# thu-pacman/chitu

Hardware: AMD Instinct MI355X
Metric: output tok/s (bs=16) DeepSeek-R1 FP8 TP=8; HBM GB/s vs peak (higher is better)
Workload: dtype fp8_e4m3 weights+activations (W8A8, fp32 accumulate), bf16 attention

## Files before the change

### chitu_amd/csrc/gate.hip

```cpp
#include "common.h"
#include "moe_align_device.h"

namespace chitu {

struct RouteAlign {
    int num_experts;
    int block_size;
    int32_t* sorted_ids;
    int64_t sorted_cap;
    int32_t* expert_ids;
    int64_t expert_cap;
    int32_t* num_post_pad;
    int32_t* cumsum;
    const int32_t* expert_map;
    unsigned int* ticket;
    int small;
};

__device__ __forceinline__ void route_align_tail(const RouteAlign& a, const int64_t* ids, int64_t numel, int* lds) {
    __shared__ int last_flag;
    asm volatile("s_waitcnt vmcnt(0)" ::: "memory");
    __syncthreads();
    if (gridDim.x == 1) {
        moe_align_workgroup<int64_t>(ids, numel, a.num_experts, a.block_size, a.sorted_ids, a.sorted_cap, a.expert_ids,
                                     a.expert_cap, a.num_post_pad, a.cumsum, 1, a.expert_map, lds, (int)blockDim.x);
        return;
    }
    if (threadIdx.x == 0) {
        __builtin_amdgcn_fence(__ATOMIC_RELEASE, "agent");
        asm volatile("s_waitcnt vmcnt(0)" ::: "memory");
        const unsigned int t = __hip_atomic_fetch_add(a.ticket, 1u, __ATOMIC_RELAXED, __HIP_MEMORY_SCOPE_AGENT);
        const int last = (t == gridDim.x - 1) ? 1 : 0;
        if (last) {
            __builtin_amdgcn_fence(__ATOMIC_ACQUIRE, "agent");
            __hip_atomic_store(a.ticket, 0u, __ATOMIC_RELAXED, __HIP_MEMORY_SCOPE_AGENT);
        }
        last_flag = last;
    }
    __syncthreads();
    if (!last_flag) return;
    moe_align_workgroup<int64_t>(ids, numel, a.num_experts, a.block_size, a.sorted_ids, a.sorted_cap, a.expert_ids,
                                 a.expert_cap, a.num_post_pad, a.cumsum, 1, a.expert_map, lds, (int)blockDim.x);
}

__device__ __forceinline__ float bf16r(float v) { return round_bf16(v); }

template <int SIGMOID>
__global__ __launch_bounds__(1024) void gate_route_kernel(
    const void* __restrict__ logits, int S, int M, int E, const bf16_t* __restrict__ bias, int n_groups,
    int topk_groups, int topk, float route_scale, bf16_t* __restrict__ out_w, int64_t* __restrict__ out_ids,
    int out_stride, int extra_id, float extra_w, int extra_n, int renorm, RouteAlign al) {
    extern __shared__ __attribute__((aligned(16))) float lds[];
    float* sc = lds;
    float* red = lds + E;
    float* gsc = lds + E + 32;
    float* wsel = lds + E + 32 + 64;
    const int t = blockIdx.x, e = threadIdx.x, lane = e & 63, wave = e >> 6;
    const int nw = blockDim.x >> 6;
    const bool act = e < E;

    float logit = -INFINITY;
    if (act) {
        if (S == 0) {
            logit = bf16_to_f32(((const bf16_t*)logits)[(int64_t)t * E + e]);
        } else {
            float a = 0.f;
            for (int s0 = 0; s0 < S; s0 += 8) {
                float v[8];
#pragma unroll
                for (int i = 0; i < 8; ++i)
                    v[i] = (s0 + i < S) ? ((const float*)logits)[((int64_t)(s0 + i) * M + t) * E + e] : 0.f;
#pragma unroll
                for (int i = 0; i < 8; ++i) a += v[i];
            }
            logit = bf16r(a);
        }
    }
    float orig;
    if (SIGMOID) {
        orig = act ? bf16r(1.0f / (1.0f + expf(-logit))) : 0.f;
    } else {
        float m = wave_reduce_max(logit);
        if (lane == 0) red[wave] = m;
        __syncthreads();
        m = red[0];
        for (int w = 1; w < nw; ++w) m = __builtin_fmaxf(m, red[w]);
        __syncthreads();
        const float ex = act ? expf(logit - m) : 0.f;
        float sum = wave_reduce_sum(ex);
        if (lane == 0) red[wave] = sum;
        __syncthreads();
        sum = 0.f;
        for (int w = 0; w < nw; ++w) sum += red[w];
        __syncthreads();
        orig = ex / sum;
    }
    float sel = orig;
    if (bias && act) sel = SIGMOID ? bf16r(orig + bf16_to_f32(bias[e])) : orig + bf16_to_f32(bias[e]);
    if (act) sc[e] = sel;
    __syncthreads();

    if (n_groups > 1) {
        const int gs = E / n_groups;
        if (gs == 32 || gs == 64) {
            const float v = act ? sel : -INFINITY;
            float m1 = v;
#pragma unroll
            for (int off = 1; off < 64; off <<= 1)
                if (off < gs) m1 = __builtin_fmaxf(m1, __shfl_xor(m1, off, 64));
            const unsigned long long gmask = gs == 64 ? ~0ull : (0xffffffffull << (lane & 32));
            const int n_max = __popcll(__ballot(v == m1) & gmask);
            float m2 = v < m1 ? v : -INFINITY;
#pragma unroll
            for (int off = 1; off < 64; off <<= 1)
                if (off < gs) m2 = __builtin_fmaxf(m2, __shfl_xor(m2, off, 64));
            if (n_max >= 2) m2 = m1;
            if (act && (e % gs) == 0) gsc[e / gs] = bias ? (SIGMOID ? bf16r(m1 + m2) : m1 + m2) : m1;
        } else if (e < n_groups) {
            float m1 = -INFINITY, m2 = -INFINITY;
            for (int i = 0; i < gs; ++i) {
                const float v = sc[e * gs + i];
                if (v > m1) { m2 = m1; m1 = v; }
                else if (v > m2) m2 = v;
            }
            gsc[e] = bias ? (SIGMOID ? bf16r(m1 + m2) : m1 + m2) : m1;
        }
        __syncthreads();
        if (act) {
            const int grp = e / gs;
            const float mine = gsc[grp];
            int rank = 0;
            for (int g2 = 0; g2 < n_groups; ++g2) {
                const float o = gsc[g2];
                rank += (o > mine) || (o == mine && g2 < grp);
            }
            if (rank >= topk_groups) sel = 0.f;
        }
        __syncthreads();
        if (act) sc[e] = sel;
        __syncthreads();
    }
    int rank = 0;
    if (act) {
        const int e4 = E & ~3;
#pragma unroll 16
        for (int i = 0; i < e4; i += 4) {
            const f32x4 o = *reinterpret_cast<const f32x4*>(&sc[i]);
            rank += (o[0] > sel) || (o[0] == sel && i < e);
            rank += (o[1] > sel) || (o[1] == sel && i + 1 < e);
            rank += (o[2] > sel) || (o[2] == sel && i + 2 < e);
            rank += (o[3] > sel) || (o[3] == sel && i + 3 < e);
        }
        for (int i = e4; i < E; ++i) {
            const float o = sc[i];
// ... 139 lines not shown
        if (lane < topk) {
            float sum = 0.f;
            for (int i = 0; i < topk; ++i) sum += wsel[i];
            float w = bf16r(wsel[lane] / bf16r(sum));
            w = bf16r(w * route_scale);
            out_w[(int64_t)t * out_stride + lane] = f32_to_bf16(w);
        }
        if (lane < extra_n && extra_id >= 0) {
            out_ids[(int64_t)t * out_stride + topk + lane] = extra_id + lane;
            out_w[(int64_t)t * out_stride + topk + lane] = f32_to_bf16(extra_w);
        }
    }
    if (al.num_experts > 0)
        route_align_tail(al, out_ids, (int64_t)M * out_stride, align_lds);
}

template <int GS>
__global__ __launch_bounds__(1024) void gate_route_align_wg_kernel(
    const void* __restrict__ logits, int S, int M, const bf16_t* __restrict__ bias, int n_groups, int topk_groups,
    int topk, float route_scale, bf16_t* __restrict__ out_w, int64_t* __restrict__ out_ids, int out_stride,
    int extra_id, float extra_w, int extra_n, RouteAlign al) {
    constexpr int E = 256;
    extern __shared__ __attribute__((aligned(16))) int dyn_lds[];
    const int nwaves = blockDim.x >> 6;
    float* orig_lds = reinterpret_cast<float*>(dyn_lds);
    int64_t* ids_lds = reinterpret_cast<int64_t*>(dyn_lds + nwaves * E);
    int* align_lds = dyn_lds + nwaves * E + 2 * ((M * out_stride + 1) & ~1);
    const int lane = threadIdx.x & 63, t = __builtin_amdgcn_readfirstlane(threadIdx.x >> 6);
    CHITU_PROBE_MARK(0);
    const bool small_sort = al.small != 0;
    if (small_sort) {
        moe_align_small_init(al.num_experts, (int64_t)M * out_stride, al.sorted_ids, al.sorted_cap, al.expert_ids, al.expert_cap,
                             align_lds, (int)threadIdx.x, (int)blockDim.x);
        __syncthreads();
    }
    if (t < M) {
        float lg[4];
        if (S == 0) {
            const i32x2 raw = *reinterpret_cast<const i32x2*>((const bf16_t*)logits + (int64_t)t * E + lane * 4);
            lg[0] = bf16_to_f32((bf16_t)((uint32_t)raw[0] & 0xffffu));
            lg[1] = bf16_to_f32((bf16_t)((uint32_t)raw[0] >> 16));
            lg[2] = bf16_to_f32((bf16_t)((uint32_t)raw[1] & 0xffffu));
            lg[3] = bf16_to_f32((bf16_t)((uint32_t)raw[1] >> 16));
        } else {
            f32x4 v[16];
#pragma unroll
            for (int i = 0; i < 16; ++i)
                v[i] = *reinterpret_cast<const f32x4*>((const float*)logits + ((int64_t)min(i, S - 1) * M + t) * E + lane * 4);
            f32x4 a = f32x4{0.f, 0.f, 0.f, 0.f};
#pragma unroll
            for (int i = 0; i < 16; ++i)
#pragma unroll
                for (int c = 0; c < 4; ++c) a[c] += i < S ? v[i][c] : 0.f;
#pragma unroll
            for (int c = 0; c < 4; ++c) lg[c] = bf16r(a[c]);
        }
        float bv[4] = {0.f, 0.f, 0.f, 0.f};
        if (bias) {
            const i32x2 raw = *reinterpret_cast<const i32x2*>(bias + lane * 4);
            bv[0] = bf16_to_f32((bf16_t)((uint32_t)raw[0] & 0xffffu));
            bv[1] = bf16_to_f32((bf16_t)((uint32_t)raw[0] >> 16));
            bv[2] = bf16_to_f32((bf16_t)((uint32_t)raw[1] & 0xffffu));
            bv[3] = bf16_to_f32((bf16_t)((uint32_t)raw[1] >> 16));
        }
        float orig[4], sel[4];
        uint32_t key[4];
        if (lg[0] == 12345.678f) CHITU_PROBE_MARK(9);
        CHITU_PROBE_MARK(1);
#pragma unroll
        for (int c = 0; c < 4; ++c) {
            orig[c] = bf16r(1.0f / (1.0f + expf(-lg[c])));
            sel[c] = bias ? bf16r(orig[c] + bv[c]) : orig[c];
            key[c] = score_key(sel[c], lane * 4 + c);
        }
        *reinterpret_cast<f32x4*>(&orig_lds[t * E + lane * 4]) = f32x4{orig[0], orig[1], orig[2], orig[3]};
        if (key[0] == 0xdeadbeefu) CHITU_PROBE_MARK(9);
        CHITU_PROBE_MARK(5);
        if (GS == 32) {
            const uint32_t k1 = group8_max_u32(max(max(key[0], key[1]), max(key[2], key[3])));
            uint32_t k2 = 0u;
#pragma unroll
            for (int c = 0; c < 4; ++c) k2 = max(k2, key[c] == k1 ? 0u : key[c]);
            k2 = group8_max_u32(k2);
            const float m1 = key_score(k1), m2 = key_score(k2);
            const float mine = bias ? bf16r(m1 + m2) : m1;
            const int grp = lane >> 3;
            int rank = 0;
#pragma unroll
            for (int g2 = 0; g2 < 8; ++g2) {
                const float o = __int_as_float(__builtin_amdgcn_readlane(__float_as_int(mine), g2 * 8));
                rank += (g2 < n_groups) && ((o > mine) || (o == mine && g2 < grp));
            }
            if (rank >= topk_groups) {
#pragma unroll
                for (int c = 0; c < 4; ++c) key[c] = score_key(0.f, lane * 4 + c);
            }
        }
        if (key[0] == 0xdeadbeefu) CHITU_PROBE_MARK(9);
        CHITU_PROBE_MARK(6);
        uint32_t mine_k = 0u;
        for (int r = 0; r < topk; ++r) {
            const uint32_t m = wave_max_u32_uniform(max(max(key[0], key[1]), max(key[2], key[3])));
            if (lane == r) mine_k = m;
#pragma unroll
            for (int c = 0; c < 4; ++c)
                if (key[c] == m) key[c] = 0u;
        }
        if (mine_k == 0xdeadbeefu) CHITU_PROBE_MARK(9);
        CHITU_PROBE_MARK(7);
        __builtin_amdgcn_fence(__ATOMIC_ACQ_REL, "wavefront");
        __builtin_amdgcn_wave_barrier();
        const int we = 0xffff - (int)(mine_k & 0xffffu);
        const float ws = lane < topk ? orig_lds[t * E + (we & (E - 1))] : 0.f;
        float sum = 0.f;
        if (topk <= 16) {
#pragma unroll
            for (int i = 0; i < 16; ++i)
                if (i < topk) sum += __int_as_float(__builtin_amdgcn_readlane(__float_as_int(ws), i));
        } else {
            for (int i = 0; i < topk; ++i) sum += __shfl(ws, i, 64);
        }
        if (lane < topk) {
            float w = bf16r(ws / bf16r(sum));
            w = bf16r(w * route_scale);
            out_w[(int64_t)t * out_stride + lane] = f32_to_bf16(w);
            out_ids[(int64_t)t * out_stride + lane] = we;
            ids_lds[t * out_stride + lane] = we;
            if (small_sort) moe_align_small_mark(align_lds, we, t);
        }
        if (lane < extra_n && extra_id >= 0) {
            out_ids[(int64_t)t * out_stride + topk + lane] = extra_id + lane;
            out_w[(int64_t)t * out_stride + topk + lane] = f32_to_bf16(extra_w);
            ids_lds[t * out_stride + topk + lane] = extra_id + lane;
            if (small_sort) moe_align_small_mark(align_lds, extra_id + lane, t);
        }
    }
    CHITU_PROBE_MARK(2);
    __syncthreads();
    CHITU_PROBE_MARK(3);
    const int sort_waves = min((int)(blockDim.x >> 6), max((al.num_experts + 63) >> 6, (M * out_stride + 63) >> 6));
    if (t >= sort_waves) return;
    if (small_sort) {
        moe_align_small_tail(ids_lds, M * out_stride, out_stride, al.num_experts, al.block_size, al.sorted_ids, al.sorted_cap,
                             al.expert_ids, al.expert_cap, al.num_post_pad, al.cumsum, al.expert_map, align_lds, sort_waves * 64);
        CHITU_PROBE_MARK(4);
        return;
    }
    moe_align_workgroup<int64_t>(ids_lds, (int64_t)M * out_stride, al.num_experts, al.block_size, al.sorted_ids,
                                 al.sorted_cap, al.expert_ids, al.expert_cap, al.num_post_pad, al.cumsum, 1,
                                 al.expert_map, align_lds, sort_waves * 64);
    CHITU_PROBE_MARK(4);
}

__device__ __forceinline__ uint32_t ordered_u32(float v) {
    const uint32_t b = __float_as_uint(v);
    return b ^ ((b & 0x80000000u) ? 0xffffffffu : 0x80000000u);
}

__global__ __launch_bounds__(1024) void gate_route_align_wg_softmax_kernel(
    const void* __restrict__ logits, int S, int M, int E, const bf16_t* __restrict__ bias, int topk, float route_scale,
    bf16_t* __restrict__ out_w, int64_t* __restrict__ out_ids, int out_stride, int extra_id, float extra_w, int extra_n,
    int renorm, RouteAlign al) {
    extern __shared__ __attribute__((aligned(16))) int dyn_lds[];
    int64_t* ids_lds = reinterpret_cast<int64_t*>(dyn_lds);
    int* align_lds = dyn_lds + 2 * ((M * out_stride + 1) & ~1);
    const int lane = threadIdx.x & 63, t = __builtin_amdgcn_readfirstlane(threadIdx.x >> 6);
    const bool small_sort = al.small != 0;
    if (small_sort) {
        moe_align_small_init(al.num_experts, (int64_t)M * out_stride, al.sorted_ids, al.sorted_cap, al.expert_ids, al.expert_cap,
                             align_lds, (int)threadIdx.x, (int)blockDim.x);
        __syncthreads();
    }
    if (t < M) {
        const bool act = lane < E;
        const int ec = act ? lane : E - 1;
        float logit;
        if (S == 0) {
            logit = bf16_to_f32(((const bf16_t*)logits)[(int64_t)t * E + ec]);
        } else {
            float v[16];
#pragma unroll
            for (int i = 0; i < 16; ++i) v[i] = ((const float*)logits)[((int64_t)min(i, S - 1) * M + t) * E + ec];
            float a = 0.f;
#pragma unroll
            for (int i = 0; i < 16; ++i) a += i < S ? v[i] : 0.f;
            logit = bf16r(a);
        }
        const float bv = bias ? bf16_to_f32(bias[ec]) : 0.f;
        if (!act) logit = -INFINITY;
        const float m = wave_reduce_max(logit);
        const float ex = act ? expf(logit - m) : 0.f;
        const float sum = wave_reduce_sum(ex);
        const float orig = ex / sum;
        const float sel = bias ? orig + bv : orig;
        uint32_t key = act ? ordered_u32(sel) : 0u;
        int my_e = 0;
        float my_w = 0.f;
        for (int r = 0; r < topk; ++r) {
            const uint32_t mk = wave_max_u32_uniform(key);
            const unsigned long long hit = __ballot(act && key == mk);
            const int win = __builtin_amdgcn_readfirstlane(__ffsll((long long)hit) - 1);
            const float w = __int_as_float(__builtin_amdgcn_readlane(__float_as_int(orig), win));
            if (lane == r) {
                my_e = win;
                my_w = w;
            }
            if (lane == win) key = 0u;
        }
        float w = my_w;
        if (renorm) {
            float s2 = 0.f;
#pragma unroll
            for (int i = 0; i < 16; ++i)
                if (i < topk) s2 += __int_as_float(__builtin_amdgcn_readlane(__float_as_int(my_w), i));
            w = w / s2;
        }
        w = w * route_scale;
        if (lane < topk) {
            out_w[(int64_t)t * out_stride + lane] = f32_to_bf16(w);
            out_ids[(int64_t)t * out_stride + lane] = my_e;
            ids_lds[t * out_stride + lane] = my_e;
            if (small_sort) moe_align_small_mark(align_lds, my_e, t);
        }
        if (lane < extra_n && extra_id >= 0) {
            out_ids[(int64_t)t * out_stride + topk + lane] = extra_id + lane;
            out_w[(int64_t)t * out_stride + topk + lane] = f32_to_bf16(extra_w);
            ids_lds[t * out_stride + topk + lane] = extra_id + lane;
            if (small_sort) moe_align_small_mark(align_lds, extra_id + lane, t);
        }
    }
    __syncthreads();
    const int sort_waves = min((int)(blockDim.x >> 6), max((al.num_experts + 63) >> 6, (M * out_stride + 63) >> 6));
    if (t >= sort_waves) return;
    if (small_sort) {
        moe_align_small_tail(ids_lds, M * out_stride, out_stride, al.num_experts, al.block_size, al.sorted_ids, al.sorted_cap,
                             al.expert_ids, al.expert_cap, al.num_post_pad, al.cumsum, al.expert_map, align_lds, sort_waves * 64);
        return;
    }
    moe_align_workgroup<int64_t>(ids_lds, (int64_t)M * out_stride, al.num_experts, al.block_size, al.sorted_ids,
                                 al.sorted_cap, al.expert_ids, al.expert_cap, al.num_post_pad, al.cumsum, 1,
                                 al.expert_map, align_lds, sort_waves * 64);
}

}

static int gate_route_launch(const void* logits, int32_t num_partials, int64_t tokens, int32_t num_experts,
                             const void* bias_bf16, int32_t n_groups, int32_t topk_groups, int32_t topk,
                             int32_t score_func, float route_scale, void* out_weights_bf16, int64_t* out_ids,
                             int32_t out_stride, int32_t extra_expert_id, float extra_weight,
                             int32_t extra_count, const chitu::RouteAlign& al, void* stream) {
    using namespace chitu;
    CHITU_REQUIRE(logits && out_weights_bf16 && out_ids && tokens >= 0);
    CHITU_REQUIRE(num_experts >= 1 && num_experts <= 1024 && topk >= 1 && topk <= num_experts && topk <= 64);
    CHITU_REQUIRE(n_groups >= 1 && n_groups <= 64 && num_experts % n_groups == 0);
    CHITU_REQUIRE(topk_groups >= 1 && topk_groups <= n_groups && num_partials >= 0);
    CHITU_REQUIRE(extra_count >= 0 && extra_count <= 32 && out_stride >= topk + (extra_expert_id >= 0 ? extra_count : 0));
    CHITU_REQUIRE(score_func >= 0 && score_func <= 2);
    if (tokens == 0) return CHITU_OK;
    const int threads = ((max(num_experts, al.num_experts) + 63) / 64) * 64;
    CHITU_REQUIRE(threads <= 1024);
    const size_t align_lds = al.num_experts > 0 ? sizeof(int) * moe_align_lds_ints(al.num_experts, threads) : 0;
    const size_t lds = max(sizeof(float) * (size_t)(num_experts + 32 + 64 + 64), align_lds);
    CHITU_REQUIRE(lds <= 60 * 1024);
    hipStream_t st = (hipStream_t)stream;
    const int gs = n_groups > 1 ? num_experts / n_groups : 0;
    const bool fast = score_func == 1 && (gs == 0 || gs == 32 || gs == 64) && num_partials <= 16 &&
                      (threads / 64) * topk <= 64 && ((threads / 64) * topk) % 4 == 0 && n_groups <= 32 &&
                      debug_option(kOptGateGeneric) <= 0;
    if (fast && al.num_experts > 0 && num_experts == 256 && (gs == 0 || gs == 32) && tokens <= 16 &&
        extra_count <= 32 && debug_option(kOptGateTicket) <= 0) {
        const int wg_threads = 64 * max((int)tokens, (max(num_experts, al.num_experts) + 63) / 64);
        const size_t ids_ints = 2 * (((size_t)tokens * out_stride + 1) & ~(size_t)1);
        const size_t wg_lds = sizeof(int) * ((size_t)(wg_threads / 64) * 256 + ids_ints +
                                             moe_align_lds_ints(al.num_experts, wg_threads));
        CHITU_REQUIRE(wg_threads <= 1024 && wg_lds <= 64 * 1024);
        RouteAlign alw = al;
        alw.small = (num_experts <= al.num_experts &&
                     (extra_expert_id < 0 || (extra_expert_id >= num_experts && extra_expert_id + extra_count <= al.num_experts)) &&
                     debug_option(kOptGateSmallSort) != 0) ? 1 : 0;
#define LAUNCHW(GSV)                                                                                          \
    hipLaunchKernelGGL(gate_route_align_wg_kernel<GSV>, dim3(1), dim3(wg_threads), wg_lds, st, logits,         \
                       (int)num_partials, (int)tokens, (const bf16_t*)bias_bf16, (int)n_groups, (int)topk_groups, \
                       (int)topk, route_scale, (bf16_t*)out_weights_bf16, out_ids, (int)out_stride,           \
                       (int)extra_expert_id, extra_weight, (int)extra_count, alw)
        if (gs == 32) LAUNCHW(32);
        else LAUNCHW(0);
#undef LAUNCHW
        CHITU_RETURN_LAUNCH_STATUS();
    }
    if (!fast && al.num_experts > 0 && num_experts <= 64 && (score_func == 0 || score_func == 2) && n_groups <= 1 &&
        tokens <= 16 && num_partials <= 16 && topk <= 16 && extra_count <= 32 && debug_option(kOptGateTicket) <= 0 &&
        debug_option(kOptGateGeneric) <= 0) {
        const int wg_threads = 64 * max((int)tokens, (max(num_experts, al.num_experts) + 63) / 64);
        const size_t ids_ints = 2 * (((size_t)tokens * out_stride + 1) & ~(size_t)1);
        const size_t wg_lds = sizeof(int) * (ids_ints + moe_align_lds_ints(al.num_experts, wg_threads));
        CHITU_REQUIRE(wg_threads <= 1024 && wg_lds <= 64 * 1024);
        RouteAlign alw = al;
        alw.small = (num_experts <= al.num_experts &&
                     (extra_expert_id < 0 || (extra_expert_id >= num_experts && extra_expert_id + extra_count <= al.num_experts)) &&
                     debug_option(kOptGateSmallSort) != 0) ? 1 : 0;
        hipLaunchKernelGGL(gate_route_align_wg_softmax_kernel, dim3(1), dim3(wg_threads), wg_lds, st, logits, (int)num_partials,
                           (int)tokens, (int)num_experts, (const bf16_t*)bias_bf16, (int)topk, route_scale,
                           (bf16_t*)out_weights_bf16, out_ids, (int)out_stride, (int)extra_expert_id, extra_weight,
                           (int)extra_count, score_func == 2 ? 1 : 0, alw);
        CHITU_RETURN_LAUNCH_STATUS();
    }
    if (fast) {
#define LAUNCHF(GSV)                                                                                         \
    hipLaunchKernelGGL(gate_route_fast_kernel<GSV>, dim3((unsigned)tokens), dim3(threads), align_lds, st, logits, \
                       (int)num_partials, (int)tokens, (int)num_experts, (const bf16_t*)bias_bf16, (int)n_groups, \
                       (int)topk_groups, (int)topk, route_scale, (bf16_t*)out_weights_bf16, out_ids,         \
                       (int)out_stride, (int)extra_expert_id, extra_weight, (int)extra_count, al)
        if (gs == 32) LAUNCHF(32);
        else if (gs == 64) LAUNCHF(64);
        else LAUNCHF(0);
#undef LAUNCHF
        CHITU_RETURN_LAUNCH_STATUS();
    }
    if (lds > 48 * 1024) {
        (void)hipFuncSetAttribute((const void*)gate_route_kernel<1>, hipFuncAttributeMaxDynamicSharedMemorySize, (int)lds);
        (void)hipFuncSetAttribute((const void*)gate_route_kernel<0>, hipFuncAttributeMaxDynamicSharedMemorySize, (int)lds);
    }
    if (score_func == 1)
        hipLaunchKernelGGL(gate_route_kernel<1>, dim3((unsigned)tokens), dim3(threads), lds, st, logits,
                           (int)num_partials, (int)tokens, (int)num_experts, (const bf16_t*)bias_bf16,
                           (int)n_groups, (int)topk_groups, (int)topk, route_scale, (bf16_t*)out_weights_bf16,
                           out_ids, (int)out_stride, (int)extra_expert_id, extra_weight, (int)extra_count, 0, al);
    else
        hipLaunchKernelGGL(gate_route_kernel<0>, dim3((unsigned)tokens), dim3(threads), lds, st, logits,
                           (int)num_partials, (int)tokens, (int)num_experts, (const bf16_t*)bias_bf16,
                           (int)n_groups, (int)topk_groups, (int)topk, route_scale, (bf16_t*)out_weights_bf16,
                           out_ids, (int)out_stride, (int)extra_expert_id, extra_weight, (int)extra_count,
                           score_func == 2 ? 1 : 0, al);
    CHITU_RETURN_LAUNCH_STATUS();
}

extern "C" int chitu_hip_gate_route(const void* logits, int32_t num_partials, int64_t tokens,
                                    int32_t num_experts, const void* bias_bf16, int32_t n_groups,
                                    int32_t topk_groups, int32_t topk, int32_t score_func,
                                    float route_scale, void* out_weights_bf16, int64_t* out_ids,
                                    int32_t out_stride, int32_t extra_expert_id, float extra_weight,
                                    int32_t extra_count, void* stream) {
    chitu::RouteAlign none{};
    return gate_route_launch(logits, num_partials, tokens, num_experts, bias_bf16, n_groups, topk_groups, topk,
                             score_func, route_scale, out_weights_bf16, out_ids, out_stride, extra_expert_id,
                             extra_weight, extra_count, none, stream);
}

extern "C" int chitu_hip_gate_route_align(const void* logits, int32_t num_partials, int64_t tokens,
                                          int32_t num_experts, const void* bias_bf16, int32_t n_groups,
                                          int32_t topk_groups, int32_t topk, int32_t score_func,
                                          float route_scale, void* out_weights_bf16, int64_t* out_ids,
                                          int32_t out_stride, int32_t extra_expert_id, float extra_weight,
                                          int32_t extra_count, int32_t align_num_experts, int32_t align_block_size,
                                          int32_t* sorted_token_ids, int64_t sorted_cap, int32_t* expert_ids,
                                          int64_t expert_ids_cap, int32_t* num_tokens_post_pad, int32_t* cumsum,
                                          const int32_t* expert_map, uint32_t* ticket, void* stream) {
    CHITU_REQUIRE(sorted_token_ids && expert_ids && num_tokens_post_pad && cumsum && ticket);
    CHITU_REQUIRE(align_num_experts >= 1 && align_num_experts <= 1024 && align_block_size >= 1);
    CHITU_REQUIRE(sorted_cap >= 0 && expert_ids_cap >= 0 && tokens * (int64_t)out_stride < (1ll << 31));
    CHITU_REQUIRE(out_stride == topk + (extra_expert_id >= 0 ? extra_count : 0));
    chitu::RouteAlign al{align_num_experts, align_block_size, sorted_token_ids, sorted_cap, expert_ids, expert_ids_cap,
                         num_tokens_post_pad, cumsum, expert_map, ticket, 0};
    return gate_route_launch(logits, num_partials, tokens, num_experts, bias_bf16, n_groups, topk_groups, topk,
                             score_func, route_scale, out_weights_bf16, out_ids, out_stride, extra_expert_id,
                             extra_weight, extra_count, al, stream);
}

CHITU_PROBE_READER(gate)
```

### chitu_amd/csrc/moe.hip

```cpp
#include "common.h"
#include "gemm_common.h"
#ifndef CHITU_MOE_PROBE_MASK
#define CHITU_MOE_PROBE_MASK 0
#endif

namespace chitu {

struct MoeStage {
    W8Frag w;
    i32x4 x[2];
    float xs, ws;
};


template <int WK, int NW, int D>
__global__ __launch_bounds__(64 * WK * NW) void moe_gemm1_kernel(
    const fp8_t* __restrict__ Xq, const float* __restrict__ Xs, const fp8_t* __restrict__ W,
    const float* __restrict__ Ws, const int32_t* __restrict__ sorted_ids,
    const int32_t* __restrict__ expert_ids, const int32_t* __restrict__ num_post_pad,
    bf16_t* __restrict__ out, int numel, int topk, int N, int K) {
    static_assert(WK == 1 || NW == 1, "either split K or tile N inside a workgroup");
    __shared__ float red[WK > 1 ? WK * 256 : 1];
    const int mb = blockIdx.y;
    if (mb * 16 >= *num_post_pad) return;
    const int lane = threadIdx.x & 63, wave = __builtin_amdgcn_readfirstlane(threadIdx.x >> 6);
    const int j = lane & 15, g = lane >> 4;
    const int n0 = (NW > 1 ? blockIdx.x * NW + wave : blockIdx.x) * 16;
    if (NW > 1 && n0 >= N) return;
    const int KB = K >> 7;
    const int slot = sorted_ids[mb * 16 + j];
    const bool valid = slot < numel;
    const int e = expert_ids[mb];
    f32x4 acc = f32x4{0.f, 0.f, 0.f, 0.f};
    if (e >= 0) {
        const int kw = NW > 1 ? 0 : wave;
        const int kb0 = KB * kw / WK, kb1 = KB * (kw + 1) / WK;
        const int slot0 = __builtin_amdgcn_readfirstlane(slot);
        const int token = (valid ? slot : min(slot0, numel - 1)) / topk;
        const fp8_t* xp = Xq + (size_t)token * K + g * 16;
        const float* xsp = Xs + (size_t)token * KB;
        const fp8_t *wp0, *wp1;
        w8_lane_ptrs(W + (size_t)e * N * K, n0, N, K, j, g, wp0, wp1);
        const float* wsp = Ws + ((size_t)e * ((N + 127) >> 7) + (n0 >> 7)) * KB;
        auto load = [&](MoeStage& st, int kb) {
            const int off = kb << 7;
            st.w.w[0] = __builtin_nontemporal_load(reinterpret_cast<const i32x4*>(wp0 + off));
            st.w.w[1] = __builtin_nontemporal_load(reinterpret_cast<const i32x4*>(wp1 + off));
            st.x[0] = *reinterpret_cast<const i32x4*>(xp + off);
            st.x[1] = *reinterpret_cast<const i32x4*>(xp + off + 64);
            st.xs = xsp[kb];
            st.ws = wsp[kb];
        };
        auto compute = [&](const MoeStage& st) {
            const f32x4 blk = w8a8_block_dot(st.w, st.x[0], st.x[1]);
#pragma unroll
            for (int r = 0; r < 4; ++r) acc[r] += (blk[r] * st.xs) * st.ws;
        };
        MoeStage ring[D];
#pragma unroll
        for (int d = 0; d < D; ++d)
            if (kb0 + d < kb1) load(ring[d], kb0 + d);
        for (int kb = kb0; kb < kb1; kb += D) {
#pragma unroll
            for (int d = 0; d < D; ++d) {
                if (kb + d < kb1) {
                    compute(ring[d]);
                    if (kb + d + D < kb1) load(ring[d], kb + d + D);
                }
            }
        }
    }
    if (WK > 1) {
        *reinterpret_cast<f32x4*>(&red[(wave * 64 + lane) * 4]) = acc;
        __syncthreads();
        if (wave != 0) return;
        acc = f32x4{0.f, 0.f, 0.f, 0.f};
#pragma unroll
        for (int w = 0; w < WK; ++w) {
            const f32x4 v = *reinterpret_cast<const f32x4*>(&red[(w * 64 + lane) * 4]);
#pragma unroll
            for (int r = 0; r < 4; ++r) acc[r] += v[r];
        }
    }
    if (!valid) return;
    moe_store_tile(out + (size_t)slot * N, n0, g, N, acc, 1.0f);
}

struct MoeStage2 {
    W8Frag wg, wu;
    i32x4 x[2];
    float xs, wsg, wsu;
};

template <int WK, int D, bool Q = false>
__global__ __launch_bounds__(Q ? 512 : 64 * WK) void moe_gemm1_silu_kernel(
    const fp8_t* __restrict__ Xq, const float* __restrict__ Xs, const fp8_t* __restrict__ W,
    const float* __restrict__ Ws, const int32_t* __restrict__ sorted_ids,
    const int32_t* __restrict__ expert_ids, const int32_t* __restrict__ num_post_pad,
    bf16_t* __restrict__ out, int numel, int topk, int I, int K, fp8_t* __restrict__ hq = nullptr,
    float* __restrict__ hs = nullptr, float eps = 0.f) {
    static_assert(!Q || WK == 1, "the quantising epilogue owns whole K");
    __shared__ float red[WK > 1 ? WK * 512 : 1];
    __shared__ float qmax[Q ? 8 * 16 : 1];
    const int mb = blockIdx.y;
    if (mb * 16 >= *num_post_pad) return;
    const int lane = threadIdx.x & 63;
    const int wave_id = __builtin_amdgcn_readfirstlane(threadIdx.x >> 6);
    const int wave = Q ? 0 : wave_id;
    const int j = lane & 15, g = lane >> 4;
    const int n0 = (Q ? blockIdx.x * 8 + wave_id : blockIdx.x) * 16;
    const int N = 2 * I;
    const int KB = K >> 7;
    const int slot = sorted_ids[mb * 16 + j];
    const bool valid = slot < numel;
    const int e = expert_ids[mb];
    f32x4 ag = f32x4{0.f, 0.f, 0.f, 0.f}, au = f32x4{0.f, 0.f, 0.f, 0.f};
    if (e >= 0) {
        const int kb0 = KB * wave / WK, kb1 = KB * (wave + 1) / WK;
        const int slot0 = __builtin_amdgcn_readfirstlane(slot);
        const int token = (valid ? slot : min(slot0, numel - 1)) / topk;
        const fp8_t* xp = Xq + (size_t)token * K + g * 16;
        const float* xsp = Xs + (size_t)token * KB;
        if (CHITU_MOE_PROBE_MASK & 1) {
            xp = Xq + (size_t)(g * 16 + (token & 15)) * 16;
            xsp = Xs + (token & 15);
        }
        const fp8_t* Wb = W + (size_t)e * N * K;
        const fp8_t *gp0, *gp1, *up0, *up1;
        w8_lane_ptrs(Wb, n0, N, K, j, g, gp0, gp1);
        w8_lane_ptrs(Wb, I + n0, N, K, j, g, up0, up1);
        const float* wsb = Ws + (size_t)e * ((N + 127) >> 7) * KB;
        const float* wsgp = wsb + (size_t)(n0 >> 7) * KB;
        const float* wsup = wsb + (size_t)((I + n0) >> 7) * KB;
        auto load = [&](MoeStage2& st, int kb) {
            const int off = kb << 7;
            st.wg.w[0] = __builtin_nontemporal_load(reinterpret_cast<const i32x4*>(gp0 + off));
            st.wg.w[1] = __builtin_nontemporal_load(reinterpret_cast<const i32x4*>(gp1 + off));
            st.wu.w[0] = __builtin_nontemporal_load(reinterpret_cast<const i32x4*>(up0 + off));
            st.wu.w[1] = __builtin_nontemporal_load(reinterpret_cast<const i32x4*>(up1 + off));
            if (CHITU_MOE_PROBE_MASK & 1) {
                st.x[0] = *reinterpret_cast<const i32x4*>(xp + (size_t)kb * 2048);
                st.x[1] = *reinterpret_cast<const i32x4*>(xp + (size_t)kb * 2048 + 1024);
                st.xs = xsp[kb * 16];
            } else {
                st.x[0] = *reinterpret_cast<const i32x4*>(xp + off);
                st.x[1] = *reinterpret_cast<const i32x4*>(xp + off + 64);
                st.xs = xsp[kb];
            }
            st.wsg = wsgp[kb];
            st.wsu = wsup[kb];
        };
        auto compute = [&](const MoeStage2& st) {
            const f32x4 bg = w8a8_block_dot(st.wg, st.x[0], st.x[1]);
            const f32x4 bu = w8a8_block_dot(st.wu, st.x[0], st.x[1]);
#pragma unroll
            for (int r = 0; r < 4; ++r) {
                ag[r] += (bg[r] * st.xs) * st.wsg;
                au[r] += (bu[r] * st.xs) * st.wsu;
            }
        };
        MoeStage2 ring[D];
#pragma unroll
        for (int d = 0; d < D; ++d)
            if (kb0 + d < kb1) load(ring[d], kb0 + d);
        for (int kb = kb0; kb < kb1; kb += D) {
#pragma unroll
            for (int d = 0; d < D; ++d) {
                if (kb + d < kb1) {
                    compute(ring[d]);
                    if (kb + d + D < kb1) load(ring[d], kb + d + D);
                }
            }
        }
    }
    if (WK > 1) {
        *reinterpret_cast<f32x4*>(&red[(wave * 128 + lane) * 4]) = ag;
        *reinterpret_cast<f32x4*>(&red[(wave * 128 + 64 + lane) * 4]) = au;
        __syncthreads();
        if (wave != 0) return;
        ag = f32x4{0.f, 0.f, 0.f, 0.f};
        au = f32x4{0.f, 0.f, 0.f, 0.f};
#pragma unroll
        for (int w = 0; w < WK; ++w) {
            const f32x4 vg = *reinterpret_cast<const f32x4*>(&red[(w * 128 + lane) * 4]);
            const f32x4 vu = *reinterpret_cast<const f32x4*>(&red[(w * 128 + 64 + lane) * 4]);
#pragma unroll
            for (int r = 0; r < 4; ++r) {
                ag[r] += vg[r];
                au[r] += vu[r];
            }
        }
    }
    if (!Q && !valid) return;
    f32x4 h;
#pragma unroll
    for (int r = 0; r < 4; ++r) {
        const float gv = round_bf16(ag[r]), uv = round_bf16(au[r]);
        const float sl = round_bf16(gv / (1.0f + expf(-gv)));
        h[r] = round_bf16(sl * uv);
    }
    if (!Q) {
        moe_store_tile(out + (size_t)slot * I, n0, g, I, h, 1.0f);
        return;
    }
    float amax = __builtin_fmaxf(__builtin_fmaxf(__builtin_fabsf(h[0]), __builtin_fabsf(h[1])),
                                 __builtin_fmaxf(__builtin_fabsf(h[2]), __builtin_fabsf(h[3])));
    amax = __builtin_fmaxf(amax, __shfl_xor(amax, 16, 64));
    amax = __builtin_fmaxf(amax, __shfl_xor(amax, 32, 64));
    if (g == 0) qmax[wave_id * 16 + j] = amax;
    __syncthreads();
    amax = qmax[j];
#pragma unroll
    for (int w = 1; w < 8; ++w) amax = __builtin_fmaxf(amax, qmax[w * 16 + j]);
    const float sc = __builtin_fmaxf(amax, eps) / 448.0f;
    const float v[8] = {h[0], h[1], h[2], h[3], 0.f, 0.f, 0.f, 0.f};
    const uint32_t codes = (uint32_t)quant8_fp8<true>(v, sc)[0];
    if (!valid) return;
    fp8_t* qrow = hq + (size_t)slot * I + n0 + 2 * g;
    *reinterpret_cast<uint16_t*>(qrow) = (uint16_t)(codes & 0xffffu);
    *reinterpret_cast<uint16_t*>(qrow + 8) = (uint16_t)(codes >> 16);
    if (wave_id == 0 && g == 0) hs[(size_t)slot * (I >> 7) + blockIdx.x] = sc;
}

__global__ __launch_bounds__(256) void moe_silu_quant_kernel(const bf16_t* __restrict__ c1,
                                                             fp8_t* __restrict__ q,
                                                             float* __restrict__ s, int64_t rows,
                                                             int I, float eps, int act_rule) {
    const int lane16 = threadIdx.x & 15;
    const int gpr = I >> 7;
    const int64_t n_groups = rows * gpr;
    int64_t group = ((int64_t)blockIdx.x * blockDim.x + threadIdx.x) >> 4;
    const int64_t stride = ((int64_t)gridDim.x * blockDim.x) >> 4;
    for (; group < n_groups; group += stride) {
        const int64_t row = group / gpr;
        const int col = (int)(group % gpr) * 128 + lane16 * 8;
        const i32x4 graw = *reinterpret_cast<const i32x4*>(c1 + row * 2 * I + col);
        const i32x4 uraw = *reinterpret_cast<const i32x4*>(c1 + row * 2 * I + I + col);
        float h[8];
        float amax = 0.f;
#pragma unroll
        for (int i = 0; i < 8; ++i) {
            const uint32_t gu = (uint32_t)graw[i >> 1], uu = (uint32_t)uraw[i >> 1];
            const float gv = (i & 1) ? __uint_as_float(gu & 0xffff0000u) : __uint_as_float(gu << 16);
            const float uv = (i & 1) ? __uint_as_float(uu & 0xffff0000u) : __uint_as_float(uu << 16);
            const float sl = round_bf16(gv / (1.0f + expf(-gv)));
            h[i] = round_bf16(sl * uv);
            amax = __builtin_fmaxf(amax, __builtin_fabsf(h[i]));
        }
        amax = row16_reduce_max(amax);
        if (!act_rule) amax = __builtin_fmaxf(amax, eps);
        const float sc = amax / 448.0f;
        const i32x2 o = act_rule ? quant8_fp8<false>(h, sc) : quant8_fp8<true>(h, sc);
        *reinterpret_cast<i32x2*>(q + row * I + col) = o;
        if (lane16 == 0) s[group] = sc;
    }
}

template <int KBMAX, int NT>
__global__ __launch_bounds__(256) void moe_gemm2_kernel(
    const fp8_t* __restrict__ Hq, const float* __restrict__ Hs, const fp8_t* __restrict__ W,
    const float* __restrict__ Ws, const int32_t* __restrict__ sorted_ids,
    const int32_t* __restrict__ expert_ids, const int32_t* __restrict__ num_post_pad,
    const void* __restrict__ topk_w, int w_dt, bf16_t* __restrict__ out, int numel, int N, int I,
    int mul_weight) {
    const int mb = blockIdx.y;
    if (mb * 16 >= *num_post_pad) return;
    const int lane = threadIdx.x & 63, wave = __builtin_amdgcn_readfirstlane(threadIdx.x >> 6);
    const int j = lane & 15, g = lane >> 4;
    const int KB = I >> 7;
    const int slot = sorted_ids[mb * 16 + j];
    const bool valid = slot < numel;
    const int e = expert_ids[mb];
    const int row = valid ? slot : 0;
    const float rw = (mul_weight && valid) ? moe_routed_weight(topk_w, w_dt, slot) : 1.0f;
    i32x4 x[KBMAX][2];
    float xs[KBMAX];
    if (e >= 0) {
        const fp8_t* xp = Hq + (size_t)row * I + g * 16;
#pragma unroll
        for (int kb = 0; kb < KBMAX; ++kb) {
            if (kb < KB) {
                x[kb][0] = *reinterpret_cast<const i32x4*>(xp + (kb << 7));
                x[kb][1] = *reinterpret_cast<const i32x4*>(xp + (kb << 7) + 64);
                xs[kb] = Hs[(size_t)row * KB + kb];
            }
        }
    }
    const int tile0 = (blockIdx.x * 4 + wave) * NT;
    W8Frag wf[NT][KBMAX];
    if (e >= 0) {
#pragma unroll
        for (int t = 0; t < NT; ++t) {
            const int n0 = (tile0 + t) * 16;
            if (n0 < N) {
                const fp8_t *wp0, *wp1;
                w8_lane_ptrs(W + (size_t)e * N * I, n0, N, I, j, g, wp0, wp1);
#pragma unroll
                for (int kb = 0; kb < KBMAX; ++kb) {
                    if (kb < KB) {
                        wf[t][kb].w[0] = __builtin_nontemporal_load(reinterpret_cast<const i32x4*>(wp0 + (kb << 7)));
                        wf[t][kb].w[1] = __builtin_nontemporal_load(reinterpret_cast<const i32x4*>(wp1 + (kb << 7)));
                    }
                }
            }
        }
    }
#pragma unroll
    for (int t = 0; t < NT; ++t) {
        const int n0 = (tile0 + t) * 16;
        if (n0 >= N) break;
        f32x4 acc = f32x4{0.f, 0.f, 0.f, 0.f};
        if (e >= 0) {
            const float* wsp = Ws + ((size_t)e * ((N + 127) >> 7) + (n0 >> 7)) * KB;
#pragma unroll
            for (int kb = 0; kb < KBMAX; ++kb) {
                if (kb < KB) {
                    const f32x4 blk = w8a8_block_dot(wf[t][kb], x[kb][0], x[kb][1]);
                    const float ws = wsp[kb];
#pragma unroll
                    for (int r = 0; r < 4; ++r) acc[r] += (blk[r] * xs[kb]) * ws;
                }
            }
        }
        if (valid) moe_store_tile(out + (size_t)slot * N, n0, g, N, acc, rw);
    }
}

template <int KB, int NT, int ROUNDS>
__global__ __launch_bounds__(256) void moe_gemm2_q_kernel(
    const bf16_t* __restrict__ Hb, const fp8_t* __restrict__ W, const float* __restrict__ Ws,
    const int32_t* __restrict__ sorted_ids, const int32_t* __restrict__ expert_ids,
    const int32_t* __restrict__ num_post_pad, const void* __restrict__ topk_w, int w_dt,
    bf16_t* __restrict__ out, int numel, int N, int mul_weight, float eps) {
    constexpr int I = KB * 128;
    constexpr int HPW = (2 * KB + 3) / 4;
    __shared__ float amax_lds[2 * KB][16];
    __shared__ i32x4 xq_lds[2 * KB][64];
    const int mb = blockIdx.y;
    if (mb * 16 >= *num_post_pad) return;
    const int lane = threadIdx.x & 63, wave = __builtin_amdgcn_readfirstlane(threadIdx.x >> 6);
    const int j = lane & 15, g = lane >> 4;
    const int slot = sorted_ids[mb * 16 + j];
    const bool valid = slot < numel;
    const int e = expert_ids[mb];
    auto tile_of = [&](int r) { return ((blockIdx.x * ROUNDS + r) * 4 + wave) * NT; };
    if (e < 0) {
#pragma unroll
        for (int r = 0; r < ROUNDS; ++r)
#pragma unroll
            for (int t = 0; t < NT; ++t) {
                const int n0 = (tile_of(r) + t) * 16;
                if (n0 < N && valid) moe_store_tile(out + (size_t)slot * N, n0, g, N, f32x4{0.f, 0.f, 0.f, 0.f}, 1.0f);
            }
        return;
    }
    const int row = valid ? slot : 0;
    const bf16_t* hrow = Hb + (size_t)row * I;
    i32x4 hraw[HPW][2];
#pragma unroll
    for (int q = 0; q < HPW; ++q) {
        const int hb = min(wave + 4 * q, 2 * KB - 1);
        hraw[q][0] = *reinterpret_cast<const i32x4*>(hrow + hb * 64 + g * 16);
        hraw[q][1] = *reinterpret_cast<const i32x4*>(hrow + hb * 64 + g * 16 + 8);
    }
    const int last_tile = (N - 1) >> 4;
    const fp8_t* We = W + (size_t)e * N * I;
    W8Frag wf[ROUNDS > 1 ? 2 : 1][NT][KB];
    auto load_round = [&](W8Frag (&dst)[NT][KB], int r) {
#pragma unroll
        for (int t = 0; t < NT; ++t) {
            const int n0 = min(tile_of(r) + t, last_tile) * 16;
            const fp8_t *wp0, *wp1;
            w8_lane_ptrs(We, n0, N, I, j, g, wp0, wp1);
#pragma unroll
            for (int kb = 0; kb < KB; ++kb) {
                dst[t][kb].w[0] = __builtin_nontemporal_load(reinterpret_cast<const i32x4*>(wp0 + (kb << 7)));
                dst[t][kb].w[1] = __builtin_nontemporal_load(reinterpret_cast<const i32x4*>(wp1 + (kb << 7)));
            }
        }
    };
    load_round(wf[0], 0);
    const float rw = (mul_weight && valid) ? moe_routed_weight(topk_w, w_dt, slot) : 1.0f;
    float h[HPW][16];
#pragma unroll
    for (int q = 0; q < HPW; ++q) {
        const int hb = wave + 4 * q;
        float amax = 0.f;
#pragma unroll
        for (int i = 0; i < 16; ++i) {
            const uint32_t u = (uint32_t)hraw[q][i >> 3][(i >> 1) & 3];
            h[q][i] = (i & 1) ? __uint_as_float(u & 0xffff0000u) : __uint_as_float(u << 16);
            amax = __builtin_fmaxf(amax, __builtin_fabsf(h[q][i]));
        }
        amax = __builtin_fmaxf(amax, __shfl_xor(amax, 16, 64));
        amax = __builtin_fmaxf(amax, __shfl_xor(amax, 32, 64));
        if (g == 0 && hb < 2 * KB) amax_lds[hb][j] = amax;
    }
    __syncthreads();
#pragma unroll
    for (int q = 0; q < HPW; ++q) {
        const int hb = wave + 4 * q;
        if (hb < 2 * KB) {
            const float sc = __builtin_fmaxf(__builtin_fmaxf(amax_lds[hb & ~1][j], amax_lds[hb | 1][j]), eps) / 448.0f;
            float lo[8], hi[8];
#pragma unroll
            for (int i = 0; i < 8; ++i) {
                lo[i] = h[q][i];
                hi[i] = h[q][8 + i];
            }
            const i32x2 a = quant8_fp8<true>(lo, sc), b = quant8_fp8<true>(hi, sc);
            xq_lds[hb][lane] = i32x4{a[0], a[1], b[0], b[1]};
        }
    }
    __syncthreads();
    i32x4 x[KB][2];
    float xs[KB];
#pragma unroll
    for (int kb = 0; kb < KB; ++kb) {
        x[kb][0] = xq_lds[2 * kb][lane];
        x[kb][1] = xq_lds[2 * kb + 1][lane];
        xs[kb] = __builtin_fmaxf(__builtin_fmaxf(amax_lds[2 * kb][j], amax_lds[2 * kb + 1][j]), eps) / 448.0f;
    }
    const float* wse = Ws + (size_t)e * ((N + 127) >> 7) * KB;
#pragma unroll
    for (int r = 0; r < ROUNDS; ++r) {
        if (r + 1 < ROUNDS) load_round(wf[(r + 1) & 1], r + 1);
#pragma unroll
        for (int t = 0; t < NT; ++t) {
            const int n0 = (tile_of(r) + t) * 16;
            f32x4 acc = f32x4{0.f, 0.f, 0.f, 0.f};
            const float* wsp = wse + (size_t)(min(n0, N - 1) >> 7) * KB;
#pragma unroll
            for (int kb = 0; kb < KB; ++kb) {
                const f32x4 blk = w8a8_block_dot(wf[r & 1][t][kb], x[kb][0], x[kb][1]);
                const float ws = wsp[kb];
#pragma unroll
                for (int rr = 0; rr < 4; ++rr) acc[rr] += (blk[rr] * xs[kb]) * ws;
            }
            if (valid && n0 < N) moe_store_tile(out + (size_t)slot * N, n0, g, N, acc, rw);
        }
    }
}

template <int WK>
__global__ __launch_bounds__(64 * WK) void moe_gemm2_generic_kernel(
    const fp8_t* __restrict__ Hq, const float* __restrict__ Hs, const fp8_t* __restrict__ W,
    const float* __restrict__ Ws, const int32_t* __restrict__ sorted_ids,
    const int32_t* __restrict__ expert_ids, const int32_t* __restrict__ num_post_pad,
    const void* __restrict__ topk_w, int w_dt, bf16_t* __restrict__ out, int numel, int N, int I,
    int mul_weight) {
    __shared__ float red[WK > 1 ? WK * 256 : 1];
    const int mb = blockIdx.y;
    if (mb * 16 >= *num_post_pad) return;
    const int lane = threadIdx.x & 63, wave = __builtin_amdgcn_readfirstlane(threadIdx.x >> 6);
    const int j = lane & 15, g = lane >> 4;
    const int n0 = blockIdx.x * 16;
    const int KB = I >> 7;
    const int slot = sorted_ids[mb * 16 + j];
    const bool valid = slot < numel;
    const int e = expert_ids[mb];
    const int row = valid ? slot : 0;
    f32x4 acc = f32x4{0.f, 0.f, 0.f, 0.f};
    if (e >= 0) {
        const int kb0 = KB * wave / WK, kb1 = KB * (wave + 1) / WK;
        const fp8_t* xp = Hq + (size_t)row * I + g * 16;
        const float* xsp = Hs + (size_t)row * KB;
        const fp8_t *wp0, *wp1;
        w8_lane_ptrs(W + (size_t)e * N * I, n0, N, I, j, g, wp0, wp1);
        const float* wsp = Ws + ((size_t)e * ((N + 127) >> 7) + (n0 >> 7)) * KB;
        for (int kb = kb0; kb < kb1; ++kb) {
            const int off = kb << 7;
            W8Frag f;
            f.w[0] = __builtin_nontemporal_load(reinterpret_cast<const i32x4*>(wp0 + off));
            f.w[1] = __builtin_nontemporal_load(reinterpret_cast<const i32x4*>(wp1 + off));
            const i32x4 x0 = *reinterpret_cast<const i32x4*>(xp + off);
            const i32x4 x1 = *reinterpret_cast<const i32x4*>(xp + off + 64);
            const f32x4 blk = w8a8_block_dot(f, x0, x1);
            const float xs = xsp[kb], ws = wsp[kb];
#pragma unroll
            for (int r = 0; r < 4; ++r) acc[r] += (blk[r] * xs) * ws;
        }
    }
    if (WK > 1) {
        *reinterpret_cast<f32x4*>(&red[(wave * 64 + lane) * 4]) = acc;
        __syncthreads();
        if (wave != 0) return;
        acc = f32x4{0.f, 0.f, 0.f, 0.f};
#pragma unroll
        for (int w = 0; w < WK; ++w) {
            const f32x4 v = *reinterpret_cast<const f32x4*>(&red[(w * 64 + lane) * 4]);
#pragma unroll
            for (int r = 0; r < 4; ++r) acc[r] += v[r];
        }
    }
    if (!valid) return;
    const float rw = mul_weight ? moe_routed_weight(topk_w, w_dt, slot) : 1.0f;
    moe_store_tile(out + (size_t)slot * N, n0, g, N, acc, rw);
}

__global__ __launch_bounds__(256) void moe_sum_kernel(const bf16_t* __restrict__ c3,
                                                      bf16_t* __restrict__ out, int64_t M, int topk,
                                                      int64_t N) {
    const int64_t n8 = N >> 3;
    for (int64_t idx = (int64_t)blockIdx.x * blockDim.x + threadIdx.x; idx < M * n8;
         idx += (int64_t)gridDim.x * blockDim.x) {
        const int64_t t = idx / n8, c = (idx % n8) * 8;
        float acc[8] = {0.f, 0.f, 0.f, 0.f, 0.f, 0.f, 0.f, 0.f};
        for (int k = 0; k < topk; ++k) {
// ... 57 lines not shown
#undef LAUNCH
    CHITU_RETURN_LAUNCH_STATUS();
}

extern "C" int chitu_hip_moe_silu_mul_quant_fp8(const void* c1_bf16, int64_t rows,
                                                int64_t inter_size, int32_t quant_mode, float eps,
                                                void* q_fp8, float* scales, void* stream) {
    using namespace chitu;
    CHITU_REQUIRE(c1_bf16 && q_fp8 && scales && rows >= 0 && inter_size >= 128);
    CHITU_REQUIRE(quant_mode == 0 || quant_mode == 1);
    if (inter_size % 128 != 0) return CHITU_ERR_UNSUPPORTED;
    if (rows == 0) return CHITU_OK;
    const int64_t lanes = rows * (inter_size / 128) * 16;
    int64_t blocks = (lanes + 255) / 256;
    if (blocks > 2048) blocks = 2048;
    hipLaunchKernelGGL(moe_silu_quant_kernel, dim3((unsigned)blocks), dim3(256), 0,
                       (hipStream_t)stream, (const bf16_t*)c1_bf16, (fp8_t*)q_fp8, scales, rows,
                       (int)inter_size, eps, quant_mode == 0 ? 1 : 0);
    CHITU_RETURN_LAUNCH_STATUS();
}

extern "C" int chitu_hip_moe_gemm2_fp8(const void* h_fp8, const float* h_scale, const void* w2_fp8,
                                       const float* w2_scale, const int32_t* sorted_token_ids,
                                       const int32_t* expert_ids,
                                       const int32_t* num_tokens_post_pad, const void* topk_weights,
                                       int weights_dtype, int32_t mul_routed_weight,
                                       void* out_bf16, int64_t numel, int64_t N, int64_t inter_size,
                                       int64_t max_mblocks, void* stream) {
    using namespace chitu;
    CHITU_REQUIRE(h_fp8 && h_scale && w2_fp8 && w2_scale && sorted_token_ids && expert_ids);
    CHITU_REQUIRE(num_tokens_post_pad && out_bf16 && (topk_weights || !mul_routed_weight));
    CHITU_REQUIRE(numel >= 0 && N >= 1 && inter_size >= 128 && max_mblocks >= 0);
    CHITU_REQUIRE(weights_dtype >= 0 && weights_dtype <= 2);
    if (inter_size % 128 != 0) return CHITU_ERR_UNSUPPORTED;
    if (numel == 0 || max_mblocks == 0) return CHITU_OK;
    hipStream_t st = (hipStream_t)stream;
    const int n_tiles = (int)((N + 15) / 16);
    const int KB = (int)(inter_size / 128);
    if (KB <= 4) {
        const int64_t mbs = numel < max_mblocks ? numel : max_mblocks;
#define LAUNCH2(KBM, NTV)                                                                        \
    hipLaunchKernelGGL((moe_gemm2_kernel<KBM, NTV>),                                             \
                       dim3((unsigned)((n_tiles + 4 * NTV - 1) / (4 * NTV)), (unsigned)max_mblocks), \
                       dim3(256), 0, st, (const fp8_t*)h_fp8, h_scale, (const fp8_t*)w2_fp8,     \
                       w2_scale, sorted_token_ids, expert_ids, num_tokens_post_pad, topk_weights, \
                       weights_dtype, (bf16_t*)out_bf16, (int)numel, (int)N, (int)inter_size,    \
                       (int)mul_routed_weight)
        const bool many = (int64_t)n_tiles * mbs > 8192;
        if (KB <= 2) {
            if (many) LAUNCH2(2, 4); else LAUNCH2(2, 2);
        } else {
            if (many) LAUNCH2(4, 4); else LAUNCH2(4, 2);
        }
#undef LAUNCH2
    } else {
        const dim3 grid((unsigned)n_tiles, (unsigned)max_mblocks);
        const int64_t wgs = (int64_t)n_tiles * (numel < max_mblocks ? numel : max_mblocks);
        int WK = wgs <= 512 ? 8 : wgs <= 1024 ? 4 : wgs <= 4096 ? 2 : 1;
        while (WK > 1 && WK > KB) WK >>= 1;
#define LAUNCHG(WKV)                                                                              \
    hipLaunchKernelGGL(moe_gemm2_generic_kernel<WKV>, grid, dim3(64 * WKV), 0, st,                \
                       (const fp8_t*)h_fp8, h_scale, (const fp8_t*)w2_fp8, w2_scale,              \
                       sorted_token_ids, expert_ids, num_tokens_post_pad, topk_weights,           \
                       weights_dtype, (bf16_t*)out_bf16, (int)numel, (int)N, (int)inter_size,     \
                       (int)mul_routed_weight)
        switch (WK) {
            case 8: LAUNCHG(8); break;
            case 4: LAUNCHG(4); break;
            case 2: LAUNCHG(2); break;
            default: LAUNCHG(1); break;
        }
#undef LAUNCHG
    }
    CHITU_RETURN_LAUNCH_STATUS();
}

extern "C" int chitu_hip_moe_gemm1_silu_fp8(const void* a_fp8, const float* a_scale, const void* w1_fp8,
                                            const float* w1_scale, const int32_t* sorted_token_ids,
                                            const int32_t* expert_ids, const int32_t* num_tokens_post_pad,
                                            void* h_bf16, int64_t numel, int32_t topk, int64_t inter_size,
                                            int64_t K, int64_t max_mblocks, void* stream) {
    using namespace chitu;
    CHITU_REQUIRE(a_fp8 && a_scale && w1_fp8 && w1_scale && sorted_token_ids && expert_ids);
    CHITU_REQUIRE(num_tokens_post_pad && h_bf16);
    CHITU_REQUIRE(numel >= 0 && topk >= 1 && inter_size >= 16 && K >= 128 && max_mblocks >= 0);
    if (K % 128 != 0 || inter_size % 16 != 0) return CHITU_ERR_UNSUPPORTED;
    if (numel == 0 || max_mblocks == 0) return CHITU_OK;
    const int n_tiles = (int)(inter_size / 16);
    const int64_t wgs = 2 * (int64_t)n_tiles * (numel < max_mblocks ? numel : max_mblocks);
    const int KB = (int)(K / 128);
    int WK = wgs <= 640 ? 8 : wgs <= 1536 ? 4 : wgs <= 3200 ? 2 : 1;
    debug_override(kOptMoeGemm1WK, WK);
    while (WK > 1 && WK > KB) WK >>= 1;
    int D = WK >= 4 ? 2 : 3;
    debug_override(kOptMoeGemm1D, D);
    hipStream_t st = (hipStream_t)stream;
    const dim3 grid((unsigned)n_tiles, (unsigned)max_mblocks);
#define LAUNCH1S(WKV, DV)                                                                                     \
    hipLaunchKernelGGL((moe_gemm1_silu_kernel<WKV, DV>), grid, dim3(64 * WKV), 0, st, (const fp8_t*)a_fp8, a_scale, \
                       (const fp8_t*)w1_fp8, w1_scale, sorted_token_ids, expert_ids, num_tokens_post_pad,      \
                       (bf16_t*)h_bf16, (int)numel, (int)topk, (int)inter_size, (int)K)
    if (WK == 8) { if (D == 2) LAUNCH1S(8, 2); else if (D == 3) LAUNCH1S(8, 3); else LAUNCH1S(8, 4); }
    else if (WK == 4) { if (D == 2) LAUNCH1S(4, 2); else if (D == 3) LAUNCH1S(4, 3); else LAUNCH1S(4, 4); }
    else if (WK == 2) { if (D == 4) LAUNCH1S(2, 4); else LAUNCH1S(2, 3); }
    else { if (D == 4) LAUNCH1S(1, 4); else LAUNCH1S(1, 3); }
#undef LAUNCH1S
    CHITU_RETURN_LAUNCH_STATUS();
}

extern "C" int chitu_hip_moe_gemm2_quant_fp8(const void* h_bf16, const void* w2_fp8, const float* w2_scale,
                                             const int32_t* sorted_token_ids, const int32_t* expert_ids,
                                             const int32_t* num_tokens_post_pad, const void* topk_weights,
                                             int weights_dtype, int32_t mul_routed_weight, void* out_bf16,
                                             int64_t numel, int64_t N, int64_t inter_size, int64_t max_mblocks,
                                             float eps, void* stream) {
    using namespace chitu;
    CHITU_REQUIRE(h_bf16 && w2_fp8 && w2_scale && sorted_token_ids && expert_ids);
    CHITU_REQUIRE(num_tokens_post_pad && out_bf16 && (topk_weights || !mul_routed_weight));
    CHITU_REQUIRE(numel >= 0 && N >= 1 && inter_size >= 128 && max_mblocks >= 0);
    CHITU_REQUIRE(weights_dtype >= 0 && weights_dtype <= 2);
    if (inter_size % 128 != 0 || inter_size > 512) return CHITU_ERR_UNSUPPORTED;
    if (numel == 0 || max_mblocks == 0) return CHITU_OK;
    hipStream_t st = (hipStream_t)stream;
    const int n_tiles = (int)((N + 15) / 16);
    const int KB = (int)(inter_size / 128);
    const int64_t mbs = numel < max_mblocks ? numel : max_mblocks;
#define LAUNCH2Q(KBV, NTV, RV)                                                                       \
    hipLaunchKernelGGL((moe_gemm2_q_kernel<KBV, NTV, RV>),                                           \
                       dim3((unsigned)((n_tiles + 4 * NTV * RV - 1) / (4 * NTV * RV)), (unsigned)max_mblocks), \
                       dim3(256), 0, st, (const bf16_t*)h_bf16, (const fp8_t*)w2_fp8, w2_scale,      \
                       sorted_token_ids, expert_ids, num_tokens_post_pad, topk_weights, weights_dtype, \
                       (bf16_t*)out_bf16, (int)numel, (int)N, (int)mul_routed_weight, eps)
    const bool many = (int64_t)n_tiles * mbs > 50000;
    int cfg = many ? 24 : 21;
    debug_override(kOptMoeGemm2Cfg, cfg);
    switch (KB) {
        case 1: LAUNCH2Q(1, 2, 1); break;
        case 2:
            if (cfg == 42) LAUNCH2Q(2, 4, 2);
            else if (cfg == 44) LAUNCH2Q(2, 4, 4);
            else if (cfg == 22) LAUNCH2Q(2, 2, 2);
            else if (cfg == 24) LAUNCH2Q(2, 2, 4);
            else if (cfg == 28) LAUNCH2Q(2, 2, 8);
            else if (cfg == 21) LAUNCH2Q(2, 2, 1);
            else LAUNCH2Q(2, 4, 1);
            break;
        case 3: LAUNCH2Q(3, 2, 1); break;
        default: LAUNCH2Q(4, 2, 1); break;
    }
#undef LAUNCH2Q
    CHITU_RETURN_LAUNCH_STATUS();
}

extern "C" int chitu_hip_moe_sum(const void* c3_bf16, void* out_bf16, int64_t tokens, int32_t topk,
                                 int64_t N, void* stream) {
    using namespace chitu;
    CHITU_REQUIRE(c3_bf16 && out_bf16 && tokens >= 0 && topk >= 1 && N >= 8);
    if (N % 8 != 0) return CHITU_ERR_UNSUPPORTED;
    if (tokens == 0) return CHITU_OK;
    int64_t blocks = (tokens * (N / 8) + 255) / 256;
    if (blocks > 2048) blocks = 2048;
    hipLaunchKernelGGL(moe_sum_kernel, dim3((unsigned)blocks), dim3(256), 0, (hipStream_t)stream,
                       (const bf16_t*)c3_bf16, (bf16_t*)out_bf16, tokens, (int)topk, N);
    CHITU_RETURN_LAUNCH_STATUS();
}
```

### chitu_amd/csrc/moe_align_device.h

```cpp
#pragma once
#include "common.h"

namespace chitu {

__host__ __device__ inline size_t moe_align_lds_ints(int E, int nthreads) {
    const int W = nthreads / 64;
    return (size_t)2 * E + W + (size_t)W * E;
}

template <typename id_t>
__device__ __forceinline__ void moe_align_workgroup(
    const id_t* __restrict__ ids, int64_t numel, int E, int block_size,
    int32_t* __restrict__ sorted_ids, int64_t sorted_cap, int32_t* __restrict__ expert_ids,
    int64_t expert_cap, int32_t* __restrict__ num_post_pad, int32_t* __restrict__ cumsum,
    int fill, const int32_t* __restrict__ expert_map, int* lds, const int nthreads) {
    const int nwaves = nthreads >> 6;
    int* counts = lds;
    int* cursor = lds + E;
    int* wave_tot = lds + 2 * E;
    int* wave_hist = lds + 2 * E + nwaves;

    const int tid = threadIdx.x;
    const int lane = tid & 63;
    const int wave = __builtin_amdgcn_readfirstlane(tid >> 6);
// ... 17 lines not shown
#pragma unroll
        for (int u = 0; u < 4; ++u)
            if (e4[u] >= 0 && e4[u] < E) atomicAdd(&my_hist[(int)e4[u]], 1);
    }
    __syncthreads();
    CHITU_PROBE_MARK(21);

    int padded = 0;
    if (tid < E) {
        int total = 0;
        for (int w = 0; w < nwaves; ++w) total += wave_hist[w * E + tid];
        counts[tid] = total;
        padded = ((total + block_size - 1) / block_size) * block_size;
    }
    int incl = padded;
#pragma unroll
    for (int off = 1; off < 64; off <<= 1) {
        const int up = __shfl_up(incl, off, 64);
        if (lane >= off) incl += up;
    }
    if (lane == 63) wave_tot[wave] = incl;
    __syncthreads();
    int wave_base = 0;
    for (int w = 0; w < wave; ++w) wave_base += wave_tot[w];
    incl += wave_base;
    const int start = incl - padded;
    if (tid < E) {
        const int32_t own_id = expert_map ? expert_map[tid] : (int32_t)tid;
        int run = start;
        for (int w = 0; w < nwaves; ++w) {
            const int c = wave_hist[w * E + tid];
            wave_hist[w * E + tid] = run;
            run += c;
        }
        cursor[tid] = run;
        cumsum[tid + 1] = incl;
        for (int i = start; i < incl; i += block_size) {
            const int b = i / block_size;
            if (b < expert_cap) expert_ids[b] = own_id;
        }
        if (tid == E - 1) *num_post_pad = incl;
    }
    if (tid == 0) cumsum[0] = 0;
    if (expert_map) {
        int total = 0;
        for (int w = 0; w < nwaves; ++w) total += wave_tot[w];
        const int32_t tail_id = expert_map[0];
        for (int64_t b = total / block_size + tid; b < expert_cap; b += nthreads) expert_ids[b] = tail_id;
    }
    __syncthreads();
    CHITU_PROBE_MARK(22);

    int nbits = 0;
    while ((1 << nbits) < E) ++nbits;
    for (int64_t base4 = w0; base4 < w1; base4 += 256) {
        int64_t e4[4];
#pragma unroll
        for (int u = 0; u < 4; ++u) e4[u] = base4 + 64 * u + lane < w1 ? (int64_t)ids[base4 + 64 * u + lane] : -1;
#pragma unroll
        for (int u = 0; u < 4; ++u) {
            const int64_t base = base4 + 64 * u;
            if (base >= w1) break;
            const int64_t i = base + lane;
            const int64_t e64 = e4[u];
            const bool valid = (e64 >= 0 && e64 < E);
            const int e = valid ? (int)e64 : 0;

            unsigned long long same = __ballot(valid);
            for (int b = 0; b < nbits; ++b) {
                const bool bit = (e >> b) & 1;
                const unsigned long long bal = __ballot(valid && bit);
                same &= bit ? bal : ~bal;
            }
            const unsigned long long lt = (lane == 0) ? 0ull : (~0ull >> (64 - lane));
            const int rank = __popcll(same & lt);
            int pos = 0;
            if (valid) pos = my_hist[e] + rank;
            __builtin_amdgcn_wave_barrier();
            if (valid) {
                if (rank == 0) my_hist[e] = pos + __popcll(same);
                if (pos < sorted_cap) sorted_ids[pos] = (int32_t)i;
            }
            __builtin_amdgcn_wave_barrier();
        }
    }
}

__host__ __device__ inline size_t moe_align_small_lds_ints(int E, int nthreads) { return (size_t)2 * E + nthreads / 64; }

__device__ __forceinline__ void moe_align_small_init(int E, int64_t numel, int32_t* __restrict__ sorted_ids, int64_t sorted_cap,
                                                     int32_t* __restrict__ expert_ids, int64_t expert_cap, int* lds,
                                                     int tid, int nthreads) {
    for (int i = tid; i < E; i += nthreads) lds[i] = 0;
    for (int64_t i = tid; i < sorted_cap; i += nthreads) sorted_ids[i] = (int32_t)numel;
    for (int64_t i = tid; i < expert_cap; i += nthreads) expert_ids[i] = 0;
}

__device__ __forceinline__ void moe_align_small_mark(int* lds, int e, int token) { atomicOr(&lds[e], 1 << token); }

__device__ __forceinline__ void moe_align_small_tail(
    const int64_t* __restrict__ ids_lds, int numel, int stride, int E, int block_size, int32_t* __restrict__ sorted_ids,
    int64_t sorted_cap, int32_t* __restrict__ expert_ids, int64_t expert_cap, int32_t* __restrict__ num_post_pad,
    int32_t* __restrict__ cumsum, const int32_t* __restrict__ expert_map, int* lds, const int nthreads) {
    const int nwaves = nthreads >> 6;
    int* tmask = lds;
    int* start_l = lds + E;
    int* wave_tot = lds + 2 * E;
    const int tid = threadIdx.x, lane = tid & 63;
    const int wave = __builtin_amdgcn_readfirstlane(tid >> 6);
    int padded = 0;
    if (tid < E) padded = ((__popc((unsigned)tmask[tid]) + block_size - 1) / block_size) * block_size;
    int incl = padded;
#pragma unroll
    for (int off = 1; off < 64; off <<= 1) {
        const int up = __shfl_up(incl, off, 64);
        if (lane >= off) incl += up;
    }
    if (lane == 63) wave_tot[wave] = incl;
    __syncthreads();
    int wave_base = 0, total = 0;
    for (int w = 0; w < nwaves; ++w) {
        const int t = wave_tot[w];
        if (w < wave) wave_base += t;
        total += t;
    }
    incl += wave_base;
    const int start = incl - padded;
    if (tid < E) {
        const int32_t own_id = expert_map ? expert_map[tid] : (int32_t)tid;
        start_l[tid] = start;
        cumsum[tid + 1] = incl;
        for (int i = start; i < incl; i += block_size) {
            const int b = i / block_size;
            if (b < expert_cap) expert_ids[b] = own_id;
        }
        if (tid == E - 1) *num_post_pad = incl;
    }
    if (tid == 0) cumsum[0] = 0;
    if (expert_map) {
        const int32_t tail_id = expert_map[0];
        for (int64_t b = total / block_size + tid; b < expert_cap; b += nthreads) expert_ids[b] = tail_id;
    }
    __syncthreads();
    if (tid < numel) {
        const int e = (int)ids_lds[tid];
        const int t = tid / stride;
        if (e >= 0 && e < E) {
            const int pos = start_l[e] + __popc((unsigned)tmask[e] & ((1u << t) - 1u));
            if (pos >= 0 && pos < sorted_cap) sorted_ids[pos] = (int32_t)tid;
        }
    }
}

}
```

### chitu_amd/deepseek_v3.py

```python

import math
from dataclasses import dataclass
from typing import List, Optional

import os

import torch
import torch.nn.functional as F

from . import fused_moe, graphs, ops
from . import tensor_parallel as tp
from .attn_backend import MLA_MULTI_MAX_Q, HipAttnBackend
from .cache_manager import MAX_DECODE_Q, PagedKVCacheManager, mla_kv_layout

FP8 = torch.float8_e4m3fn
BLOCK = 128


@dataclass
class DeepSeekV3Args:

    vocab_size: int = 129280
    dim: int = 7168
    inter_dim: int = 18432
# ... 187 lines not shown
        return self._w_uk_t

    def first_projection(self):
        return self.wqkv_a if self.q_lora_rank > 0 else self.wq_kv_a

    def decode_forward_paged(self, x_quant, cos, sin, first=None, q_len=1):
        H, C, R = self.n_local_heads, self.kv_lora_rank, self.qk_rope_head_dim
        if first is not None:
            bs = first.shape[0]
        else:
            bs = x_quant[0].rows if isinstance(x_quant[0], ops.TiledQuant) else x_quant[0].shape[0]
        cache = self.cache
        kv_cache = cache.get_paged_kv_cache(self.layer_id)
        if q_len > 1:
            assert bs % q_len == 0
            kv_table, kv_lens = cache.get_gpu_multi_block_table(), cache.get_gpu_multi_row_lens()
        else:
            kv_table, kv_lens = cache.get_gpu_block_table(), cache.get_gpu_seq_lens_excl_this_decode()
        paged = None
        if self.kv_fp8:
            paged = (kv_cache, kv_table, kv_lens)
            kv_cache, kv_table, kv_lens = self.kv_stage.rows, self.kv_stage.table[:bs], self.kv_stage.lens[:bs]
        nblk = C // BLOCK
        if self.q_lora_rank > 0:
            splits = _wqkv_a_splits(bs, self.wqkv_a.out_features, self.wqkv_a.in_features)
            if first is not None or isinstance(x_quant[0], ops.TiledQuant):
                splits = 1
            if first is not None:
                q_a_kv = first
            elif splits > 1:
                q_a_kv = ops.fp8_gemm_partials_deepseek_v3(x_quant[0], x_quant[1], self.wqkv_a.weight, self.wqkv_a.scale, splits)
            else:
                q_a_kv = self.wqkv_a(None, x_quant=x_quant)
            if FUSE_Q_PROJ and splits == 1 and bs <= _Q_PROJ_MAX_BS and ops.mla_q_proj_fits(bs, self.q_lora_rank):
                q = ops.mla_q_proj(q_a_kv, self.q_lora_rank, self.q_norm.weight, self.q_norm.eps, self.wq_b.weight,
                                   self.wq_b.scale, self.kv_norm.weight, self.kv_norm.eps, cos, sin, kv_cache,
                                   kv_table, kv_lens, out_dtype=torch.bfloat16)
            else:
                qq, qs = ops.mla_qkv_post(q_a_kv, self.q_lora_rank, self.q_norm.weight, self.q_norm.eps, self.kv_norm.weight,
                                          self.kv_norm.eps, cos, sin, kv_cache, kv_table, kv_lens)
                q = self.wq_b(None, x_quant=(qq, qs))
            q = q.view(bs, H, self.qk_head_dim)
            q_nope, q_pe = q[..., : self.qk_nope_head_dim], q[..., self.qk_nope_head_dim :]
            q_abs = ops.absorb_bmm_rope_fp8(q_nope, self.w_uk_transposed(), self.wkv_b.scale, 0, 2 * nblk, 1, 0, q_pe, cos, sin)
        else:
            q_kv = first if first is not None else self.wq_kv_a(None, x_quant=x_quant)
            nq = H * self.qk_head_dim
            q = q_kv[:, :nq].view(bs, H, self.qk_head_dim)
            q_nope, q_pe = q[..., : self.qk_nope_head_dim], q[..., self.qk_nope_head_dim :]
            q_abs = ops.absorb_bmm_rope_kv_fp8(q_nope, self.w_uk_transposed(), self.wkv_b.scale, 0, 2 * nblk, 1, 0, q_pe, cos, sin,
                                               q_kv[:, nq:], self.kv_norm.weight, self.kv_norm.eps, kv_cache,
                                               kv_table, kv_lens)
        if paged is not None:
            kv_cache = paged[0]
            ops.append_mla_kv_fp8(kv_cache, paged[1], self.kv_stage.rows[:bs], paged[2])
        fuse_merge = bs <= 32 and C == 512
        w_uv = self.wkv_b.weight.view(H, self.qk_nope_head_dim + self.v_head_dim, C)[:, self.qk_nope_head_dim :]
        if q_len == 1 and fuse_merge and _MLA_FUSED_TAIL and self.v_head_dim == 128:
            fused = self.attn_backend.mla_decode_merge_uv_quant(
                q_abs, q_pe, kv_cache, cache.get_gpu_seq_lens_incl_this_decode(), cache.get_gpu_block_table(), self.softmax_scale,
                w_uv, self.wkv_b.scale, nblk, 2 * nblk, 1, tile_major=ops.tile_major_ok(bs))
            if fused is not None:
                return self.wo(None, x_quant=fused)
        if q_len > 1:
            o = self.attn_backend.mla_decode_multi(q_abs.view(bs // q_len, q_len, H, C), q_pe.unflatten(0, (bs // q_len, q_len)), kv_cache,
                                                   cache.get_gpu_multi_seq_lens_incl(), cache.get_gpu_multi_block_table()[::q_len],
                                                   self.softmax_scale, return_partials=fuse_merge,
                                                   expanded=(cache.get_gpu_multi_block_table(), cache.get_gpu_multi_row_lens_incl()))
            if not isinstance(o, tuple):
                o = o.view(bs, H, C)
        else:
            o = self.attn_backend.mla_decode(q_abs, q_pe, kv_cache, cache.get_gpu_seq_lens_incl_this_decode(),
                                             cache.get_gpu_block_table(), self.softmax_scale, return_partials=fuse_merge)
        if isinstance(o, tuple):
            oq, os_ = ops.mla_merge_absorb_uv_quant_fp8(o[0], o[1], bs, w_uv, self.wkv_b.scale, nblk, 2 * nblk, 1,
                                                        tile_major=ops.tile_major_ok(bs))
        else:
            oq, os_ = ops.absorb_uv_quant_fp8(o, w_uv, self.wkv_b.scale, nblk, 2 * nblk, 1)
        return self.wo(None, x_quant=(oq, os_))


    def prefill_forward(self, x_quant, cos, sin, varlens):
        if getattr(varlens, "continued", False):
            return self.prefill_forward_paged(x_quant, cos, sin, varlens)
        H, C, R = self.n_local_heads, self.kv_lora_rank, self.qk_rope_head_dim
        T = x_quant[0].shape[0]
        q_abs, q_pe, kv_c, kv_pe = self._prefill_projections(x_quant, cos, sin)
        self.cache.finalize_cache_bylayer_prefill(ops.mla_kv_quant_fp8(kv_pe) if self.kv_fp8 else kv_pe, None,
                                                  self.cache.curr_req_ids, self.cache.curr_varlens, self.layer_id)
        o = self.attn_backend.attn_varlen_func(
            torch.cat([q_abs, q_pe], dim=-1), kv_pe.view(T, 1, C + R), kv_c.view(T, 1, C), varlens.prefix_lens,
            varlens.prefix_lens, varlens.max_len, varlens.max_len, causal=True, softmax_scale=self.softmax_scale)
        return self._prefill_output(o)

    def _prefill_projections(self, x_quant, cos, sin):
        H, C = self.n_local_heads, self.kv_lora_rank
        T = x_quant[0].shape[0]
        if self.q_lora_rank > 0:
            q_a_kv = self.wqkv_a(None, x_quant=x_quant)
            ql = self.q_lora_rank
            _, qq, qs = ops.rms_norm(q_a_kv[:, :ql], self.q_norm.weight, self.q_norm.eps, out_bf16=False, quant="act")
            q = self.wq_b(None, x_quant=(qq, qs)).view(T, H, self.qk_head_dim)
        else:
            q_a_kv = self.wq_kv_a(None, x_quant=x_quant)
            ql = H * self.qk_head_dim
            q = q_a_kv[:, :ql].view(T, H, self.qk_head_dim)
        q_nope, q_pe = q[..., : self.qk_nope_head_dim], q[..., self.qk_nope_head_dim :]
        kv_c = ops.rms_norm(q_a_kv[:, ql : ql + C], self.kv_norm.weight, self.kv_norm.eps)
        q_pe, k_pe = ops.apply_rotary_pos_emb(q_pe, q_a_kv[:, ql + C :], cos, sin, rotary_type="llama")
        kv_pe = torch.cat([kv_c, k_pe], dim=-1)
        nblk = C // BLOCK
        q_abs = ops.absorb_bmm_fp8(q_nope, self.w_uk_transposed(), self.wkv_b.scale, 0, 2 * nblk, 1, 0)
        return q_abs, q_pe, kv_c, kv_pe

    def _prefill_output(self, o):
        H, C = self.n_local_heads, self.kv_lora_rank
        nblk = C // BLOCK
        w_uv = self.wkv_b.weight.view(H, self.qk_nope_head_dim + self.v_head_dim, C)[:, self.qk_nope_head_dim :]
        oq, os_ = ops.absorb_uv_quant_fp8(o, w_uv, self.wkv_b.scale, nblk, 2 * nblk, 1)
        return self.wo(None, x_quant=(oq, os_))

    def prefill_forward_paged(self, x_quant, cos, sin, varlens):
        q_abs, q_pe, _, kv_pe = self._prefill_projections(x_quant, cos, sin)
        self.cache.finalize_cache_bylayer_prefill_continue(ops.mla_kv_quant_fp8(kv_pe) if self.kv_fp8 else kv_pe, None, self.layer_id)
        o = self.attn_backend.mla_attn_varlen_with_kvcache(
            torch.cat([q_abs, q_pe], dim=-1), self.cache.get_paged_kv_cache(self.layer_id), varlens.prefix_lens,
            self.cache.get_gpu_continue_seq_lens_incl(), self.cache.get_gpu_continue_block_table(), varlens.max_len,
            varlens.total_keys, self.softmax_scale, gathered=varlens.gathered)
        return self._prefill_output(o)


class MLPDeepSeekV3(torch.nn.Module):

    def __init__(self, args, device=None, inter: Optional[int] = None):
        super().__init__()
        tp_size = args.tp_degree()
        self.inter = args.inter_dim // tp_size if inter is None else inter
        self.w1w3 = Fp8Linear(args.dim, 2 * self.inter, device)
        self.w2 = Fp8Linear(self.inter, args.dim, device)

    def forward(self, x_quant):
        h = self.w1w3(None, x_quant=x_quant)
        hq, hs = fused_moe.silu_and_mul_quant(h, mode="act")
        return self.w2(None, x_quant=(hq, hs))


_ROUTE_ALIGN_MAX_TOKENS = 64


def _route_align_enabled(tokens: int) -> bool:
    return tokens <= _ROUTE_ALIGN_MAX_TOKENS and os.environ.get("CHITU_ROUTE_ALIGN", "1") != "0"


class GateDeepSeekV3(torch.nn.Module):

    def __init__(self, args, device=None):
        super().__init__()
        self.topk, self.n_groups, self.topk_groups = args.n_activated_experts, args.n_expert_groups, args.n_limited_groups
        self.score_func, self.route_scale = args.score_func, args.route_scale
        self.weight = torch.nn.Parameter(torch.empty(args.n_routed_experts, args.dim, dtype=torch.bfloat16, device=device), requires_grad=False)
        self.bias = (torch.nn.Parameter(torch.empty(args.n_routed_experts, dtype=torch.bfloat16, device=device), requires_grad=False)
                     if args.has_gate_bias() else None)

    def forward(self, x, extra_expert_id: int = -1, extra_count: int = 1, align=None, logits_partials=None):
        return ops.gate_deepseek_v3(x, self.weight, self.bias, self.n_groups, self.topk_groups, self.topk,
                                    self.score_func, self.route_scale, extra_expert_id=extra_expert_id,
                                    extra_count=extra_count, align=align, logits_partials=logits_partials)


class MoEDeepSeekV3(torch.nn.Module):

    def __init__(self, args, device=None):
        super().__init__()
        tp_size = args.tp_degree()
        self.n_routed, self.n_shared = args.n_routed_experts, args.n_shared_experts
        self.moe_world_size = args.moe_world_size
        self.gate = GateDeepSeekV3(args, device)
        if self.moe_world_size > 1:
            ep = self.moe_world_size
            assert tp_size == ep, "experts are partitioned over the ranks that share the activations (tp group)"
            assert self.n_routed % ep == 0, f"Number of experts must be divisible by world size (world_size={ep})"
            self.moe_rank = (tp.get_tp_rank() % ep) if args.moe_rank is None else args.moe_rank
            self.n_local_experts = self.n_routed // ep
            self.experts_start_idx = self.moe_rank * self.n_local_experts
            self.experts_end_idx = self.experts_start_idx + self.n_local_experts
            emap = torch.full((self.n_routed,), -1, dtype=torch.int32)
            emap[self.experts_start_idx:self.experts_end_idx] = torch.arange(self.n_local_experts, dtype=torch.int32)
            self.register_buffer("expert_map", emap.to(device) if device is not None else emap, persistent=False)
            self.inter = args.moe_inter_dim
            E = self.n_local_experts
            shared_inter = self.n_shared * args.moe_inter_dim
            assert shared_inter % (ep * BLOCK) == 0 or self.n_shared == 0, "shared width / ep must keep 128-blocks whole"
            self.shared = MLPDeepSeekV3(args, device, inter=shared_inter // ep) if self.n_shared else None
        else:
            self.inter = args.moe_inter_dim // tp_size
            E = self.n_routed + self.n_shared
        assert args.expert_dtype in ("fp8", "mxfp4"), f"unknown expert_dtype {args.expert_dtype!r}"
        self.mxfp4 = args.expert_dtype == "mxfp4"
        if self.mxfp4:
            assert args.dim % BLOCK == 0 and self.inter % BLOCK == 0, "MXFP4 experts need whole 128-blocks"
            u8 = lambda *shape: torch.nn.Parameter(torch.empty(*shape, dtype=torch.uint8, device=device), requires_grad=False)
            self.w1w3_weight, self.w1w3_scale = u8(E, 2 * self.inter, args.dim // 2), u8(E, 2 * self.inter, args.dim // 32)
            self.w2_weight, self.w2_scale = u8(E, args.dim, self.inter // 2), u8(E, args.dim, self.inter // 32)
            return
        self.w1w3_weight = torch.nn.Parameter(torch.empty(E, 2 * self.inter, args.dim, dtype=FP8, device=device), requires_grad=False)
        self.w1w3_scale = torch.nn.Parameter(torch.empty(E, (2 * self.inter + BLOCK - 1) // BLOCK, args.dim // BLOCK, dtype=torch.float32, device=device), requires_grad=False)
        self.w2_weight = torch.nn.Parameter(torch.empty(E, args.dim, self.inter, dtype=FP8, device=device), requires_grad=False)
        self.w2_scale = torch.nn.Parameter(torch.empty(E, args.dim // BLOCK, (self.inter + BLOCK - 1) // BLOCK, dtype=torch.float32, device=device), requires_grad=False)

    def forward(self, x, x_quant, defer_sum: bool = False, logits_partials=None):
        nr, ns = self.n_routed, self.n_shared
        if self.moe_world_size > 1:
            return self.forward_expert_parallel(x, x_quant)
        align = (nr + ns, fused_moe._MOE_BLOCK_M, None) if _route_align_enabled(x.shape[0]) else None
        routed = (self.gate(x, extra_expert_id=nr, extra_count=ns, align=align, logits_partials=logits_partials) if ns >= 1
                  else self.gate(x, align=align, logits_partials=logits_partials))
        weights, indices = routed[0], routed[1]
        aligned = routed[2] if len(routed) > 2 else None
        return fused_moe.fused_experts(
            x, self.w1w3_weight, self.w2_weight, topk_weights=weights, topk_ids=indices, use_fp8_w8a8=not self.mxfp4,
            inplace=True, global_num_experts=nr + ns, w1_scale=self.w1w3_scale, w2_scale=self.w2_scale,
            block_shape=[BLOCK, BLOCK], a1_quant=x_quant, reduce_topk=not defer_sum, aligned=aligned,
            use_mxfp4_w4a8=self.mxfp4,
        )

    def forward_expert_parallel(self, x, x_quant):
        align = (self.n_routed, fused_moe._MOE_BLOCK_M, self.expert_map) if _route_align_enabled(x.shape[0]) else None
        routed = self.gate(x, align=align)
        weights, indices = routed[0], routed[1]
        y = fused_moe.fused_experts(
            x, self.w1w3_weight, self.w2_weight, topk_weights=weights, topk_ids=indices, use_fp8_w8a8=not self.mxfp4,
            inplace=True, global_num_experts=self.n_routed, expert_map=self.expert_map, w1_scale=self.w1w3_scale,
            w2_scale=self.w2_scale, block_shape=[BLOCK, BLOCK], a1_quant=x_quant,
            aligned=routed[2] if len(routed) > 2 else None, use_mxfp4_w4a8=self.mxfp4,
        )
        if self.shared is not None:
            y += self.shared(x_quant)
        return y


class TransformerBlockDeepSeekV3(torch.nn.Module):

    def __init__(self, layer_id, args, cache, attn_backend, device=None, kv_stage=None):
        super().__init__()
        self.attn = AttentionDeepSeekV3(args, layer_id, cache, attn_backend, device, kv_stage)
        self.is_moe = layer_id >= args.n_dense_layers
        self.ffn = MoEDeepSeekV3(args, device) if self.is_moe else MLPDeepSeekV3(args, device)
        self.attn_norm = RMSNormW(args.dim, args.norm_eps, device)
        self.ffn_norm = RMSNormW(args.dim, args.norm_eps, device)

    def forward(self, x, pending, cos, sin, varlens=None, q_len=1):
        tm = varlens is None and pending is not None and ops.tile_major_ok(x.shape[0])
        if varlens is None and _fuses_attn_norm_into_first_projection(x, pending, self.attn):
            proj = self.attn.first_projection()
            x, first = ops.fp8_linear_add_norm(x, pending, self.attn_norm.weight, self.attn_norm.eps, proj.weight, proj.scale)
            a = tp.defer_all_reduce(self.attn.decode_forward_paged(None, cos, sin, first=first, q_len=q_len))
            return self.ffn_part(x, a, cos, sin, varlens)
        x, _, xq, xs = add_norm(x, pending, self.attn_norm, out_bf16=False, quant="act", tile_major=tm)
        if varlens is None:
            a = tp.defer_all_reduce(self.attn.decode_forward_paged((xq, xs), cos, sin, q_len=q_len))
        else:
            a = tp.defer_all_reduce(self.attn.prefill_forward((xq, xs), cos, sin, varlens))
        return self.ffn_part(x, a, cos, sin, varlens)

    def ffn_part(self, x, a, cos, sin, varlens):
        if self.is_moe:
            x, hn, hq, hs = add_norm(x, a, self.ffn_norm, out_bf16=True, quant="group")
            defer = (tp.defers_topk_sum(hn.shape[0], hn.shape[1], self.ffn.gate.topk + self.ffn.n_shared)
                     and self.ffn.moe_world_size == 1 and os.environ.get("CHITU_DEFER_TOPK_SUM", "1") != "0")
            f = self.ffn(hn, (hq, hs), defer_sum=defer)
        else:
            x, _, hq, hs = add_norm(x, a, self.ffn_norm, out_bf16=False, quant="act",
                                    tile_major=varlens is None and ops.tile_major_ok(x.shape[0]))
            f = self.ffn((hq, hs))
        return x, tp.defer_all_reduce(f)


FUSE_ATTN_NORM_MAX_BS = int(os.environ.get("CHITU_FUSE_ATTN_NORM_MAX_BS", "1"))


def _fuses_attn_norm_into_first_projection(x, pending, attn) -> bool:
    if not (isinstance(pending, torch.Tensor) and pending.dim() in (2, 3) and x.shape[0] <= FUSE_ATTN_NORM_MAX_BS):
        return False
    proj = attn.first_projection()
    terms = pending.shape[1] if pending.dim() == 3 else 1
    return (proj.weight.element_size() == 1 and os.environ.get("CHITU_WQKV_SPLIT", "0") != "1"
            and ops.fp8_linear_add_norm_fits(x.shape[0], proj.out_features, proj.in_features, terms))




def add_norm(x, pending, norm, out_bf16=True, quant=None, tile_major=False):
    return tp.add_norm(x, pending, norm.weight, norm.eps, out_bf16=out_bf16, quant=quant, tile_major=tile_major)


class DeepSeekV3Decoder(torch.nn.Module):

    def __init__(self, args: DeepSeekV3Args, cache: PagedKVCacheManager, attn_backend: HipAttnBackend,
                 max_position_embeddings: int = 4096, device="cuda", layers: Optional[List[int]] = None):
        super().__init__()
        self.args, self.cache, self.attn_backend, self.device = args, cache, attn_backend, torch.device(device)
        deg = args.tp_degree()
        assert args.vocab_size % deg == 0
        self.vocab_local = args.vocab_size // deg
        self.vocab_start = (tp.get_tp_rank() % deg) * self.vocab_local
        self.embed_weight = torch.nn.Parameter(torch.empty(self.vocab_local, args.dim, dtype=torch.bfloat16, device=device), requires_grad=False)
        ids = list(range(args.n_layers)) if layers is None else layers
        kv_shape, kv_dtype = mla_kv_layout(args.kv_cache_dtype, args.kv_lora_rank, args.qk_rope_head_dim)
        kv_stage = None
        assert args.kv_cache_dtype == "bf16" or (args.kv_lora_rank, args.qk_rope_head_dim) == (512, 64), "the fp8 KV kernels are built for 512 + 64 rows"
        if cache is not None:
            held = getattr(cache, "paged_kv_cache", None)
            matches = held is not None and held.dtype == kv_dtype and tuple(held.shape[3:]) == tuple(kv_shape)
            assert matches or (held is None and args.kv_cache_dtype == "bf16"), (
                f"kv_cache_dtype={args.kv_cache_dtype!r} needs a cache of {kv_shape} x {kv_dtype} per token "
                f"(cache_manager.mla_kv_layout), got {None if held is None else (tuple(held.shape[3:]), held.dtype)}")
            if args.kv_cache_dtype == "fp8":
                kv_stage = Fp8KvStage(cache.curr_seq_lens_gpu_excl_this_decode.shape[0], device)
        self.layers = torch.nn.ModuleList(TransformerBlockDeepSeekV3(i, args, cache, attn_backend, device, kv_stage) for i in ids)
        self.norm = RMSNormW(args.dim, args.norm_eps, device)
        self.head_weight = torch.nn.Parameter(torch.empty(self.vocab_local, args.dim, dtype=torch.bfloat16, device=device), requires_grad=False)
        cos, sin = precompute_freqs_cis(args, max_position_embeddings)
        self.cos_table, self.sin_table = cos.to(device), sin.to(device)
        self.graphs, self.static_tokens, self.static_out = {}, {}, {}
        self.graph_pool = None

    def decode_eager(self, tokens, q_len=1):
        positions = self.cache.get_gpu_multi_row_lens() if q_len > 1 else self.cache.get_gpu_seq_lens_excl_this_decode()
        h, cos, sin = ops.embed_rope_gather(tokens, self.embed_weight, self.vocab_start if self.vocab_local != self.args.vocab_size else 0,
                                            positions, self.cos_table, self.sin_table)
        if self.vocab_local != self.args.vocab_size:
            h = tp.all_reduce(h)
        pending = None
        for layer in self.layers:
            h, pending = layer(h, pending, cos, sin, q_len=q_len)
        h = add_norm(h, pending, self.norm)[1]
        return tp.all_gather_last_dim(ops.bf16_linear(h, self.head_weight), out_dtype=torch.float32)

    @torch.inference_mode()
    def prefill(self, tokens, req_ids, chunk_size=None):
        if chunk_size is not None:
            c = int(chunk_size)
            if c < 1:
                raise ValueError(f"chunk_size={chunk_size}: at least one token per round")
            req_ids = list(req_ids)
            logits = self.prefill([list(t[:c]) for t in tokens], req_ids)
            done = c
            while True:
                live = [i for i, t in enumerate(tokens) if len(t) > done]
                if not live:
                    return logits
                out = self.prefill_continue([list(tokens[i][done : done + c]) for i in live], [req_ids[i] for i in live])
                logits[torch.tensor(live, device=logits.device)] = out
                done += c

        from . import graphs

        graphs.sweep_if_memory_was_recycled()
        varlens = VarLens(tokens, self.device)
        self.cache.curr_varlens, self.cache.curr_req_ids = varlens, list(req_ids)
        flat = torch.tensor([t for seq in tokens for t in seq], dtype=torch.int64, device=self.device)
        cos, sin = self.cos_table[varlens.position_ids], self.sin_table[varlens.position_ids]
        h, pending = self.embed(flat), None
        for layer in self.layers:
            h, pending = layer(h, pending, cos, sin, varlens)
        self.cache.finalize_cache_all_prefill(req_ids, varlens)
        return self._last_token_logits(h, pending, varlens)

    def _last_token_logits(self, h, pending, varlens):
# ... 190 lines not shown
```

### chitu_amd/fused_moe.py

```python

import os
from typing import List, Optional, Tuple

import torch

from . import _lib, workspace
from ._lib import check, f32, float_dtype_code, i32, i64, int_dtype_code, ptr, require_cuda, stream_ptr

__all__ = [
    "moe_align_block_size",
    "per_token_group_quant_fp8",
    "fused_experts",
    "fused_experts_impl",
]


def ceil_div(a, b):
    return (a + b - 1) // b


def cuda_moe_align_block_size(
    topk_ids: torch.Tensor,
    num_experts: int,
    block_size: int,
    sorted_token_ids: torch.Tensor,
    experts_ids: torch.Tensor,
    num_tokens_post_pad: torch.Tensor,
    cumsum_buffer: torch.Tensor,
) -> None:
    for t in (topk_ids, sorted_token_ids, experts_ids, num_tokens_post_pad, cumsum_buffer):
        if not t.is_contiguous():
            raise RuntimeError("Tensor is not contiguous")
    require_cuda(topk_ids, sorted_token_ids, experts_ids, num_tokens_post_pad, cumsum_buffer)
    for t in (sorted_token_ids, experts_ids, num_tokens_post_pad, cumsum_buffer):
        if t.dtype != torch.int32:
            raise RuntimeError("Tensor type is incorrect")
    if cumsum_buffer.numel() < num_experts + 1:
        raise RuntimeError("cumsum_buffer too small")
    check(
        _lib.lib().chitu_hip_moe_align_block_size(
            ptr(topk_ids), int_dtype_code(topk_ids.dtype), i64(topk_ids.numel()), i32(num_experts),
            i32(block_size), ptr(sorted_token_ids), i64(sorted_token_ids.numel()), ptr(experts_ids),
            i64(experts_ids.numel()), ptr(num_tokens_post_pad), ptr(cumsum_buffer), i32(0), stream_ptr(),
        ),
        "cuda_moe_align_block_size",
    )


def _expert_map_i32(expert_map: Optional[torch.Tensor], num_experts: int, dev) -> Optional[torch.Tensor]:
    if expert_map is None:
        return None
    assert expert_map.numel() >= num_experts, "expert_map must cover every global expert id"
    if expert_map.dtype != torch.int32 or expert_map.device != dev or not expert_map.is_contiguous():
        expert_map = expert_map.to(device=dev, dtype=torch.int32).contiguous()
    return expert_map


def moe_align_block_size(
    topk_ids: torch.Tensor,
    block_size: int,
    num_experts: int,
    expert_map: torch.Tensor = None,
) -> Tuple[torch.Tensor, torch.Tensor, torch.Tensor]:
    require_cuda(topk_ids)
    if not topk_ids.is_contiguous():
        topk_ids = topk_ids.contiguous()
    numel = topk_ids.numel()
    max_num_tokens_padded = numel + num_experts * (block_size - 1)
    dev = topk_ids.device
    sorted_ids = torch.empty((max_num_tokens_padded,), dtype=torch.int32, device=dev)
    max_num_m_blocks = ceil_div(max_num_tokens_padded, block_size)
    expert_ids = torch.empty((max_num_m_blocks,), dtype=torch.int32, device=dev)
    num_tokens_post_pad = torch.empty((1), dtype=torch.int32, device=dev)
    cumsum_buffer = torch.empty((num_experts + 1,), dtype=torch.int32, device=dev)
    emap = _expert_map_i32(expert_map, num_experts, dev)
    check(
        _lib.lib().chitu_hip_moe_align_block_size_mapped(
            ptr(topk_ids), int_dtype_code(topk_ids.dtype), i64(numel), i32(num_experts), i32(block_size),
            ptr(sorted_ids), i64(sorted_ids.numel()), ptr(expert_ids), i64(expert_ids.numel()),
            ptr(num_tokens_post_pad), ptr(cumsum_buffer), i32(1), ptr(emap), stream_ptr(),
        ),
        "moe_align_block_size",
    )
    return sorted_ids, expert_ids, num_tokens_post_pad


def per_token_group_quant_fp8(
    x: torch.Tensor,
    group_size: int,
    eps: float = 1e-10,
    dtype: Optional[torch.dtype] = None,
    column_major_scales: bool = False,
) -> Tuple[torch.Tensor, torch.Tensor]:
    if dtype is None:
        dtype = torch.float8_e4m3fn
    assert dtype == torch.float8_e4m3fn, "only torch.float8_e4m3fn (OCP) is supported"
    assert x.shape[-1] % group_size == 0, (
        f"the last dimension of `x` {x.shape[-1]} must be divisible " f"by `group_size` {group_size}"
    )
    assert x.stride(-1) == 1, "`x` groups must be contiguous"
    assert not column_major_scales, "column-major scales are not used on this path"
    require_cuda(x)
    if not x.is_contiguous():
        x = x.contiguous()
    x_q = torch.empty_like(x, dtype=dtype)
    x_s = torch.empty(x.shape[:-1] + (x.shape[-1] // group_size,), device=x.device, dtype=torch.float32)
    cols = x.shape[-1]
    rows = x.numel() // cols if cols else 0
    check(
        _lib.lib().chitu_hip_act_quant_fp8(
            ptr(x), float_dtype_code(x.dtype), i64(rows), i64(cols), i32(group_size), i32(1), f32(eps),
            ptr(x_q), ptr(x_s), stream_ptr(),
        ),
        "per_token_group_quant_fp8",
    )
    return x_q, x_s


_MOE_BLOCK_M = 16
_MOE_TILED_MIN_TOKENS = int(os.environ.get("CHITU_MOE_TILED_MIN_TOKENS", "128"))
_MOE_TILED_MIN_PER_EXPERT = 24
_MOE_TILED_BLOCK_M = int(os.environ.get("CHITU_MOE_TILED_BLOCK_M", "128"))
_MOE_MXFP4_TILED_MIN_TOKENS = int(os.environ.get("CHITU_MOE_MXFP4_TILED_MIN_TOKENS", "512"))
_MOE_BF16_TILED_MIN_TOKENS = int(os.environ.get("CHITU_MOE_BF16_TILED_MIN_TOKENS", "0"))



def _takes_tiled(num_tokens, numel, global_num_experts, I, Nout, aligned, min_tokens=None):
    floor = _MOE_TILED_MIN_TOKENS if min_tokens is None else min_tokens
    return (_MOE_TILED_MIN_TOKENS > 0 and floor > 0 and num_tokens >= floor and aligned is None and I % 128 == 0
            and Nout % 8 == 0 and numel >= _MOE_TILED_MIN_PER_EXPERT * global_num_experts)

class SiluAndMul(torch.nn.Module):

    def forward(self, x: torch.Tensor) -> torch.Tensor:
        d = x.shape[-1] // 2
        return torch.nn.functional.silu(x[..., :d]) * x[..., d:]


def fused_experts(
    hidden_states: torch.Tensor,
    w1: torch.Tensor,
    w2: torch.Tensor,
    topk_weights: torch.Tensor,
    topk_ids: torch.Tensor,
    inplace: bool = False,
    activation: str = "silu",
    use_fp8_w8a8: bool = False,
    use_int8_w8a16: bool = False,
    use_int4_w4a16: bool = False,
    global_num_experts: int = -1,
    expert_map: Optional[torch.Tensor] = None,
    w1_scale: Optional[torch.Tensor] = None,
    w2_scale: Optional[torch.Tensor] = None,
    w1_zp: Optional[torch.Tensor] = None,
    w2_zp: Optional[torch.Tensor] = None,
    a1_scale: Optional[torch.Tensor] = None,
    a2_scale: Optional[torch.Tensor] = None,
    block_shape: Optional[List[int]] = None,
    soft_fp8: bool = False,
    a1_quant=None,
    reduce_topk: bool = True,
    use_int8_w8a8: bool = False,
    aligned=None,
    bf16_tiled_min_tokens: Optional[int] = None,
    use_mxfp4_w4a8: bool = False,
) -> torch.Tensor:
    return fused_experts_impl(
        hidden_states, w1, w2, topk_weights, topk_ids, inplace, activation, use_fp8_w8a8,
        use_int8_w8a16, use_int4_w4a16, global_num_experts, expert_map, w1_scale, w2_scale, w1_zp,
        w2_zp, a1_scale, a2_scale, block_shape, soft_fp8=soft_fp8, a1_quant=a1_quant, reduce_topk=reduce_topk,
        use_int8_w8a8=use_int8_w8a8, aligned=aligned, use_mxfp4_w4a8=use_mxfp4_w4a8,
        bf16_tiled_min_tokens=bf16_tiled_min_tokens,
    )


def fused_experts_impl(
    hidden_states: torch.Tensor,
    w1: torch.Tensor,
    w2: torch.Tensor,
    topk_weights: torch.Tensor,
    topk_ids: torch.Tensor,
    inplace: bool = False,
    activation: str = "silu",
    use_fp8_w8a8: bool = False,
    use_int8_w8a16: bool = False,
    use_int4_w4a16: bool = False,
    global_num_experts: int = -1,
    expert_map: Optional[torch.Tensor] = None,
    w1_scale: Optional[torch.Tensor] = None,
    w2_scale: Optional[torch.Tensor] = None,
    w1_zp: Optional[torch.Tensor] = None,
    w2_zp: Optional[torch.Tensor] = None,
    a1_scale: Optional[torch.Tensor] = None,
    a2_scale: Optional[torch.Tensor] = None,
    block_shape: Optional[List[int]] = None,
    soft_fp8: bool = False,
    a1_quant=None,
    reduce_topk: bool = True,
    use_int8_w8a8: bool = False,
    aligned=None,
    bf16_tiled_min_tokens: Optional[int] = None,
    use_mxfp4_w4a8: bool = False,
):
    if use_mxfp4_w4a8:
        if activation != "silu":
            raise ValueError(f"Unsupported FusedMoe activation: {activation}")
        return _fused_experts_mxfp4(hidden_states, w1, w2, topk_weights, topk_ids, inplace, global_num_experts, expert_map,
                                    w1_scale, w2_scale, a1_quant, reduce_topk, aligned)
    assert hidden_states.shape[1] == w1.shape[2], "Hidden size mismatch"
    assert topk_weights.shape == topk_ids.shape, "topk shape mismatch"
    assert hidden_states.is_contiguous(), "Hidden_states must be contiguous"
    assert w1.is_contiguous(), "Expert weights1 must be contiguous"
    assert w2.is_contiguous(), "Expert weights2 must be contiguous"
    assert hidden_states.dtype in [torch.float32, torch.float16, torch.bfloat16]
    if activation != "silu":
        raise ValueError(f"Unsupported FusedMoe activation: {activation}")
    if use_int8_w8a8:
        return _fused_experts_int8(hidden_states, w1, w2, topk_weights, topk_ids, inplace, global_num_experts,
                                   expert_map, w1_scale, w2_scale, reduce_topk, aligned, a1_quant)
    if use_int8_w8a16 or use_int4_w4a16:
        raise NotImplementedError(
            "chitu_amd.fused_moe implements the modes the reference's DeepSeek MoE drives (bf16 experts, fp8_w8a8 "
            "block-scaled experts with soft_fp8 on or off) and int8 W8A8 (use_int8_w8a8=True); the weight-only "
            "int8 / int4 modes are not built"
        )
    if not use_fp8_w8a8 or soft_fp8:
        return _fused_experts_bf16_act(hidden_states, w1, w2, topk_weights, topk_ids, inplace, global_num_experts,
                                       expert_map, w1_scale if use_fp8_w8a8 else None,
                                       w2_scale if use_fp8_w8a8 else None, block_shape, reduce_topk, aligned,
                                       bf16_tiled_min_tokens)
    assert block_shape is not None and list(block_shape) == [128, 128], "block_shape must be [128, 128]"
    assert w1_scale is not None and w2_scale is not None
    assert a1_scale is None and a2_scale is None, "dynamic per-token-group activation scales only"
    assert hidden_states.dtype == torch.bfloat16, "bf16 activations (the reference's R1 configuration)"
    require_cuda(hidden_states, w1, w2, topk_weights, topk_ids, w1_scale, w2_scale)
    assert w1_scale.is_contiguous() and w2_scale.is_contiguous()
    assert w1_scale.dtype == torch.float32 and w2_scale.dtype == torch.float32

    num_tokens, K = hidden_states.shape
    E, N, _ = w1.shape
    I = N // 2
    assert w2.shape[0] == E and w2.shape[2] == I, "w2 must be [E, hidden_out, N/2]"
    Nout = w2.shape[1]
    if global_num_experts == -1:
        global_num_experts = E
    topk = topk_ids.shape[1]
    dev = hidden_states.device
    out = hidden_states if inplace else torch.empty_like(hidden_states)
    if num_tokens == 0:
        return out
    numel = num_tokens * topk
    if not topk_ids.is_contiguous():
        topk_ids = topk_ids.contiguous()
    if not topk_weights.is_contiguous():
        topk_weights = topk_weights.contiguous()

    def rnd(n):
        return (n + 255) // 256 * 256

    tiled = _takes_tiled(num_tokens, numel, global_num_experts, I, Nout, aligned)
    block_m = _MOE_TILED_BLOCK_M if tiled else _MOE_BLOCK_M
    cap = numel + global_num_experts * (block_m - 1)
    nblk = ceil_div(cap, block_m)
    KB = K // 128
    sizes = [
        ("sorted", cap * 4), ("experts", nblk * 4), ("npost", 4), ("cumsum", (global_num_experts + 1) * 4),
        ("a1q", num_tokens * K), ("a1s", num_tokens * KB * 4), ("c1", numel * N * 2),
        ("a2q", numel * I), ("a2s", numel * (I // 128) * 4), ("c3", numel * Nout * 2),
    ]
    total = sum(rnd(n) for _, n in sizes)
    ws = workspace.get(total, dev, "moe")
    base = ws.data_ptr()
    off = {}
    cur = 0
    for name, n in sizes:
        off[name] = base + cur
        cur += rnd(n)
    import ctypes as _ct

    P = lambda name: _ct.c_void_p(off[name])
    lib = _lib.lib()
    st = stream_ptr()
    max_mblocks = min(nblk, numel)

    if aligned is None:
        emap = _expert_map_i32(expert_map, global_num_experts, dev)
        check(
            lib.chitu_hip_moe_align_block_size_mapped(
                ptr(topk_ids), int_dtype_code(topk_ids.dtype), i64(numel), i32(global_num_experts),
                i32(block_m), P("sorted"), i64(cap), P("experts"), i64(nblk), P("npost"), P("cumsum"),
                i32(1), ptr(emap), st,
            ),
            "moe_align_block_size",
        )
        sorted_p, experts_ptr, npost_p = P("sorted"), P("experts"), P("npost")
    else:
        a_sorted, a_experts, a_npost = aligned
        require_cuda(a_sorted, a_experts, a_npost)
        assert a_sorted.dtype == torch.int32 and a_experts.dtype == torch.int32 and a_npost.dtype == torch.int32
        assert a_sorted.numel() == cap and a_experts.numel() == nblk, "aligned buffers must come from block 16 over global_num_experts"
        sorted_p, experts_ptr, npost_p = ptr(a_sorted), ptr(a_experts), ptr(a_npost)
    if a1_quant is None:
        check(
            lib.chitu_hip_act_quant_fp8(
                ptr(hidden_states), float_dtype_code(hidden_states.dtype), i64(num_tokens), i64(K), i32(128),
                i32(1), f32(1e-10), P("a1q"), P("a1s"), st,
            ),
            "moe quant1",
        )
        a1q_p, a1s_p = P("a1q"), P("a1s")
    else:
        aq, as_ = a1_quant
        assert aq.is_contiguous() and as_.is_contiguous() and aq.numel() == num_tokens * K
        assert as_.dtype == torch.float32 and as_.numel() == num_tokens * KB
        a1q_p, a1s_p = ptr(aq), ptr(as_)
    if tiled:
        assert nblk <= 65535
        check(
            lib.chitu_hip_moe_gemm1_silu_fp8_tiled(
                a1q_p, a1s_p, ptr(w1), ptr(w1_scale), sorted_p, experts_ptr, npost_p, P("c1"),
                i64(numel), i32(topk), i64(I), i64(K), i64(max_mblocks), i32(block_m), st,
            ),
            "moe gemm1 (tiled, silu fused)",
        )
        check(
            lib.chitu_hip_act_quant_fp8(P("c1"), float_dtype_code(torch.bfloat16), i64(numel), i64(I), i32(128), i32(1),
                                        f32(1e-10), P("a2q"), P("a2s"), st),
            "moe quant2",
        )
        check(
            lib.chitu_hip_moe_gemm2_fp8_tiled(
                P("a2q"), P("a2s"), ptr(w2), ptr(w2_scale), sorted_p, experts_ptr, npost_p,
                ptr(topk_weights), float_dtype_code(topk_weights.dtype), i32(1), P("c3"), i64(numel), i64(Nout),
                i64(I), i64(max_mblocks), i32(block_m), st,
            ),
            "moe gemm2 (tiled)",
        )
    elif I % 128 == 0 and I <= 512 and os.environ.get("CHITU_MOE_FUSE_SILU", "1") != "0":
        check(
            lib.chitu_hip_moe_gemm1_silu_fp8(
                a1q_p, a1s_p, ptr(w1), ptr(w1_scale), sorted_p, experts_ptr, npost_p, P("c1"),
                i64(numel), i32(topk), i64(I), i64(K), i64(max_mblocks), st,
            ),
            "moe gemm1 (silu fused)",
        )
        check(
            lib.chitu_hip_moe_gemm2_quant_fp8(
                P("c1"), ptr(w2), ptr(w2_scale), sorted_p, experts_ptr, npost_p, ptr(topk_weights),
                float_dtype_code(topk_weights.dtype), i32(1), P("c3"), i64(numel), i64(Nout), i64(I),
                i64(max_mblocks), f32(1e-10), st,
            ),
            "moe gemm2 (quant fused)",
        )
    else:
        check(
            lib.chitu_hip_moe_gemm1_fp8(
                a1q_p, a1s_p, ptr(w1), ptr(w1_scale), sorted_p, experts_ptr, npost_p, P("c1"),
                i64(numel), i32(topk), i64(N), i64(K), i64(max_mblocks), st,
            ),
            "moe gemm1",
        )
        check(
            lib.chitu_hip_moe_silu_mul_quant_fp8(P("c1"), i64(numel), i64(I), i32(1), f32(1e-10), P("a2q"), P("a2s"), st),
            "moe silu_mul_quant",
        )
        check(
            lib.chitu_hip_moe_gemm2_fp8(
                P("a2q"), P("a2s"), ptr(w2), ptr(w2_scale), sorted_p, experts_ptr, npost_p,
                ptr(topk_weights), float_dtype_code(topk_weights.dtype), i32(1), P("c3"), i64(numel), i64(Nout),
                i64(I), i64(max_mblocks), st,
            ),
            "moe gemm2",
        )
    if not reduce_topk:
        c3_off = off["c3"] - base
        return ws[c3_off : c3_off + numel * Nout * 2].view(torch.bfloat16).view(num_tokens, topk, Nout)
    check(lib.chitu_hip_moe_sum(P("c3"), ptr(out), i64(num_tokens), i32(topk), i64(Nout), st), "moe sum")
    return out


def _fused_experts_mxfp4(hidden_states, w1, w2, topk_weights, topk_ids, inplace, global_num_experts, expert_map,
                         w1_scale, w2_scale, a1_quant, reduce_topk, aligned):
    assert topk_weights.shape == topk_ids.shape, "topk shape mismatch"
    assert hidden_states.dim() == 2 and hidden_states.is_contiguous(), "Hidden_states must be contiguous"
    assert hidden_states.dtype == torch.bfloat16, "bf16 activations"
    assert w1_scale is not None and w2_scale is not None, "MXFP4 experts need their E8M0 scales"
    for t in (w1, w2, w1_scale, w2_scale):
        assert t.dtype == torch.uint8 and t.is_contiguous() and t.dim() == 3, "MXFP4 weights and scales are contiguous uint8 [E, rows, .]"
    num_tokens, K = hidden_states.shape
    E, N, _ = w1.shape
    I = N // 2
    Nout = w2.shape[1]
    assert K % 128 == 0 and I % 128 == 0 and N == 2 * I, "K and the expert width must be multiples of 128"
    assert tuple(w1.shape) == (E, N, K // 2) and tuple(w1_scale.shape) == (E, N, K // 32), "w1 [E, 2I, K/2], w1_scale [E, 2I, K/32]"
    assert tuple(w2.shape) == (E, Nout, I // 2) and tuple(w2_scale.shape) == (E, Nout, I // 32), "w2 [E, Nout, I/2], w2_scale [E, Nout, I/32]"
    require_cuda(hidden_states, w1, w2, topk_weights, topk_ids, w1_scale, w2_scale)
    if global_num_experts == -1:
        global_num_experts = E
    topk = topk_ids.shape[1]
    dev = hidden_states.device
    out = hidden_states if inplace else torch.empty_like(hidden_states)
    if num_tokens == 0:
        return out
    assert Nout == K or not reduce_topk, "the summed output has the hidden size"
    numel = num_tokens * topk
    topk_ids = topk_ids.contiguous()
    topk_weights = topk_weights.contiguous()
    tiled = _takes_tiled(num_tokens, numel, global_num_experts, I, Nout, aligned, min_tokens=_MOE_MXFP4_TILED_MIN_TOKENS)
    block_m = _MOE_TILED_BLOCK_M if tiled else _MOE_BLOCK_M
    cap = numel + global_num_experts * (block_m - 1)
    nblk = ceil_div(cap, block_m)
    KB = K // 128
    rnd = lambda n: (n + 255) // 256 * 256
    sizes = [("sorted", cap * 4), ("experts", nblk * 4), ("npost", 4), ("cumsum", (global_num_experts + 1) * 4),
             ("a1q", num_tokens * K), ("a1s", num_tokens * KB * 4), ("c1", numel * N * 2),
             ("a2q", numel * I), ("a2s", numel * (I // 128) * 4), ("c3", numel * Nout * 2)]
    ws = workspace.get(sum(rnd(n) for _, n in sizes), dev, "moe")
    base, off, cur = ws.data_ptr(), {}, 0
    for name, n in sizes:
        off[name] = base + cur
        cur += rnd(n)
    import ctypes as _ct

    P = lambda name: _ct.c_void_p(off[name])
    lib, st = _lib.lib(), stream_ptr()
    max_mblocks = min(nblk, numel)
    if aligned is None:
        emap = _expert_map_i32(expert_map, global_num_experts, dev)
        check(lib.chitu_hip_moe_align_block_size_mapped(ptr(topk_ids), int_dtype_code(topk_ids.dtype), i64(numel),
                                                        i32(global_num_experts), i32(block_m), P("sorted"), i64(cap),
                                                        P("experts"), i64(nblk), P("npost"), P("cumsum"), i32(1), ptr(emap), st),
              "moe_align_block_size")
        sorted_p, experts_p, npost_p = P("sorted"), P("experts"), P("npost")
    else:
        a_sorted, a_experts, a_npost = aligned
        require_cuda(a_sorted, a_experts, a_npost)
        assert a_sorted.dtype == torch.int32 and a_experts.dtype == torch.int32 and a_npost.dtype == torch.int32
        assert a_sorted.numel() == cap and a_experts.numel() == nblk, "aligned buffers must come from block 16 over global_num_experts"
        sorted_p, experts_p, npost_p = ptr(a_sorted), ptr(a_experts), ptr(a_npost)
    if a1_quant is None:
        check(lib.chitu_hip_act_quant_fp8(ptr(hidden_states), float_dtype_code(hidden_states.dtype), i64(num_tokens), i64(K),
                                          i32(128), i32(1), f32(1e-10), P("a1q"), P("a1s"), st), "moe quant1")
        a1q_p, a1s_p = P("a1q"), P("a1s")
    else:
        aq, as_ = a1_quant
        require_cuda(aq, as_)
        assert aq.is_contiguous() and as_.is_contiguous() and aq.element_size() == 1 and aq.numel() == num_tokens * K
        assert as_.dtype == torch.float32 and as_.numel() == num_tokens * KB
        a1q_p, a1s_p = ptr(aq), ptr(as_)
    wdt = float_dtype_code(topk_weights.dtype)
    if tiled:
        assert nblk <= 65535
        check(lib.chitu_hip_moe_gemm1_silu_mxfp4_tiled(a1q_p, a1s_p, ptr(w1), ptr(w1_scale), sorted_p, experts_p, npost_p, P("c1"),
                                                       i64(numel), i32(topk), i64(I), i64(K), i64(max_mblocks), i32(block_m), st),
              "moe mxfp4 gemm1 (tiled, silu fused)")
        check(lib.chitu_hip_act_quant_fp8(P("c1"), float_dtype_code(torch.bfloat16), i64(numel), i64(I), i32(128), i32(1),
                                          f32(1e-10), P("a2q"), P("a2s"), st), "moe quant2")
        check(lib.chitu_hip_moe_gemm2_mxfp4_tiled(P("a2q"), P("a2s"), ptr(w2), ptr(w2_scale), sorted_p, experts_p, npost_p,
                                                  ptr(topk_weights), i32(wdt), i32(1), P("c3"), i64(numel), i64(Nout), i64(I),
                                                  i64(max_mblocks), i32(block_m), st), "moe mxfp4 gemm2 (tiled)")
    elif I <= 512:
        check(lib.chitu_hip_moe_gemm1_silu_mxfp4(a1q_p, a1s_p, ptr(w1), ptr(w1_scale), sorted_p, experts_p, npost_p, P("c1"),
                                                 i64(numel), i32(topk), i64(I), i64(K), i64(max_mblocks), st),
              "moe mxfp4 gemm1 (silu fused)")
        check(lib.chitu_hip_moe_gemm2_quant_mxfp4(P("c1"), ptr(w2), ptr(w2_scale), sorted_p, experts_p, npost_p,
                                                  ptr(topk_weights), i32(wdt), i32(1), P("c3"), i64(numel), i64(Nout), i64(I),
                                                  i64(max_mblocks), f32(1e-10), st), "moe mxfp4 gemm2 (quant fused)")
    else:
        check(lib.chitu_hip_moe_gemm_mxfp4(a1q_p, a1s_p, i32(topk), ptr(w1), ptr(w1_scale), sorted_p, experts_p, npost_p,
# ... 187 lines not shown
```

### chitu_amd/ops.py

```python

import os as _os
from typing import Tuple

import torch

from . import _lib, workspace
from ._lib import check, f32, float_dtype_code, i32, i64, ptr, require_cuda, stream_ptr

__all__ = [
    "append_to_paged_kv_cache",
    "apply_rotary_pos_emb",
    "apply_rotary_pos_emb_torch",
    "act_quant_deepseek_v3",
    "weight_dequant_deepseek_v3",
    "weight_dequant_soft_fp8_deepseek_v3",
    "fp8_gemm_deepseek_v3",
    "soft_fp8_gemm_deepseek_v3",
]

_GEMM_WS_BYTES = 64 << 20
_TILE_MAJOR_MAX_ROWS = 64
_TILE_MAJOR = _os.environ.get("CHITU_TILE_MAJOR", "1") != "0"


# ... 602 lines not shown
        return (torch.nn.functional.silu(y[:, :inter]) * y[:, inter:]).view(*x.shape[:-1], inter)
    out = torch.empty(*x.shape[:-1], inter, dtype=torch.bfloat16, device=x.device)
    check(_lib.lib().chitu_hip_bf16_gemm_silu(ptr(x), ptr(w13), ptr(out), i64(M), i64(inter), i64(K), stream_ptr()),
          "bf16_linear_silu")
    return out


def bf16_add_norm_fits(M: int, N: int, K: int) -> bool:
    if not (1 <= M <= 4 and K % 64 == 0 and 512 <= K <= 8192 and M * K <= 24576):
        return False
    tiles, wk = (N + 15) // 16, 8
    while wk > 1 and (wk > K // 64 or tiles * wk > 4096):
        wk >>= 1
    return wk >= 4


def fp8_linear_add_norm_fits(M: int, N: int, K: int, terms: int = 1) -> bool:
    if not ((M == 1 or (M == 2 and terms == 1)) and K % 128 == 0 and 128 <= K <= 8192 and 1 <= terms <= 16):
        return False
    tiles, kb = (N + 15) // 16, K // 128
    t = max(1, min(kb, (1536 + tiles - 1) // tiles))
    wk = 1
    while wk * 2 <= t and wk < 8:
        wk *= 2
    if tiles * wk < 256 and N * K >= (24 << 20):
        return False
    while wk > 1 and wk > kb:
        wk >>= 1
    return wk >= 4


def fp8_linear_add_norm(x, add, norm_weight, eps, weight, weight_scale, out_dtype=torch.bfloat16):
    require_cuda(x, add, norm_weight, weight, weight_scale)
    assert x.dtype == torch.bfloat16 and add.dtype == torch.bfloat16 and x.dim() == 2 and x.stride(1) == 1
    assert weight.element_size() == 1 and weight_scale.dtype == torch.float32 and weight.is_contiguous() and weight_scale.is_contiguous()
    M, K = x.shape
    N = weight.shape[0]
    if add.dim() == 3:
        assert add.shape[0] == M and add.shape[2] == K and add.is_contiguous()
        terms, term_stride, add_stride = add.shape[1], K, add.shape[1] * K
    else:
        assert add.shape == x.shape and add.stride(1) == 1
        terms, term_stride, add_stride = 1, 0, add.stride(0)
    assert fp8_linear_add_norm_fits(M, N, K, terms)
    x_new = torch.empty(M, K, dtype=torch.bfloat16, device=x.device)
    out = torch.empty(M, N, dtype=out_dtype, device=x.device)
    check(
        _lib.lib().chitu_hip_fp8_gemm_add_norm(
            ptr(x), i64(x.stride(0)), ptr(add), i64(add_stride), i32(terms), i64(term_stride), ptr(x_new), i64(K),
            ptr(norm_weight), f32(eps), ptr(weight), ptr(weight_scale), ptr(out), float_dtype_code(out.dtype), i64(M), i64(N),
            i64(K), stream_ptr()),
        "fp8_linear_add_norm",
    )
    return x_new, out


def bf16_linear_add_norm(x, add, norm_weight, eps, weight, out_dtype=None):
    require_cuda(x, add, norm_weight, weight)
    assert x.dtype == torch.bfloat16 and add.dtype == torch.bfloat16 and weight.dtype == torch.bfloat16
    terms = 1
    if add.dim() == 3:
        assert add.shape[0] == x.shape[0] and add.shape[1] == 2 and add.shape[2] == x.shape[1] and add.is_contiguous()
        terms = 2
    else:
        assert add.shape == x.shape and add.stride(1) == 1
    assert x.dim() == 2 and x.stride(1) == 1 and weight.is_contiguous()
    assert norm_weight.dtype == torch.bfloat16 and norm_weight.is_contiguous() and norm_weight.numel() == x.shape[1]
    M, K = x.shape
    N = weight.shape[0]
    assert weight.shape[1] == K and bf16_add_norm_fits(M, N, K), "use rms_norm(add=) + bf16_linear for this shape"
    x_new = torch.empty(M, K, dtype=torch.bfloat16, device=x.device)
    out = torch.empty(M, N, dtype=out_dtype or torch.bfloat16, device=x.device)
    check(
        _lib.lib().chitu_hip_bf16_gemm_add_norm(ptr(x), i64(x.stride(0)), ptr(add), i64(add.stride(0)), i32(terms),
                                                i64(add.stride(1) if terms == 2 else 0), ptr(x_new), i64(K),
                                                ptr(norm_weight), f32(eps), ptr(weight), ptr(out), float_dtype_code(out.dtype),
                                                i64(M), i64(N), i64(K), stream_ptr()),
        "bf16_linear_add_norm",
    )
    return x_new, out


def bf16_linear_add_norm_qkv_post(x, add, norm_weight, eps, wqkv, q_heads, kv_heads, cos, sin, k_cache, v_cache,
                                  page_table, old_seq_lens):
    require_cuda(x, add, norm_weight, wqkv, cos, sin, k_cache, v_cache, page_table, old_seq_lens)
    assert x.dtype == torch.bfloat16 and add.dtype == torch.bfloat16 and wqkv.dtype == torch.bfloat16
    assert x.dim() == 2 and add.shape == x.shape and x.stride(1) == 1 and add.stride(1) == 1 and wqkv.is_contiguous()
    assert norm_weight.dtype == torch.bfloat16 and norm_weight.is_contiguous() and norm_weight.numel() == x.shape[1]
    M, K = x.shape
    N = wqkv.shape[0]
    d = N // (q_heads + 2 * kv_heads)
    assert N == (q_heads + 2 * kv_heads) * d and d % 16 == 0 and wqkv.shape[1] == K and bf16_add_norm_fits(M, N, K)
    assert k_cache.is_contiguous() and v_cache.is_contiguous() and k_cache.shape == v_cache.shape and k_cache.dtype == torch.bfloat16
    assert tuple(k_cache.shape[2:]) == (kv_heads, d) and page_table.dtype == torch.int32 and page_table.is_contiguous()
    assert cos.dtype == torch.float32 and cos.is_contiguous() and sin.is_contiguous() and cos.shape == (M, d // 2)
    assert old_seq_lens.dtype == torch.int32 and page_table.shape[0] >= M
    x_new = torch.empty(M, K, dtype=torch.bfloat16, device=x.device)
    qkv = torch.empty(M, q_heads + 2 * kv_heads, d, dtype=torch.bfloat16, device=x.device)
    check(
        _lib.lib().chitu_hip_bf16_gemm_add_norm_qkv_post(
            ptr(x), i64(x.stride(0)), ptr(add), i64(add.stride(0)), ptr(x_new), i64(K), ptr(norm_weight), f32(eps), ptr(wqkv),
            ptr(qkv), i64(M), i64(K), i32(q_heads), i32(kv_heads), i32(d), ptr(cos), ptr(sin), ptr(k_cache), ptr(v_cache),
            i64(k_cache.shape[0]), i32(k_cache.shape[1]), ptr(page_table), i32(page_table.shape[1]), ptr(old_seq_lens),
            stream_ptr()),
        "bf16_linear_add_norm_qkv_post",
    )
    return x_new, qkv


def bf16_linear_silu_add_norm(x, add, norm_weight, eps, w13):
    require_cuda(x, add, norm_weight, w13)
    assert x.dtype == torch.bfloat16 and add.dtype == torch.bfloat16 and w13.dtype == torch.bfloat16
    assert x.dim() == 2 and add.shape == x.shape and x.stride(1) == 1 and add.stride(1) == 1 and w13.is_contiguous()
    assert norm_weight.dtype == torch.bfloat16 and norm_weight.is_contiguous() and norm_weight.numel() == x.shape[1]
    M, K = x.shape
    inter = w13.shape[0] // 2
    assert w13.shape == (2 * inter, K) and bf16_add_norm_fits(M, inter, K), "use rms_norm(add=) + bf16_linear_silu for this shape"
    x_new = torch.empty(M, K, dtype=torch.bfloat16, device=x.device)
    out = torch.empty(M, inter, dtype=torch.bfloat16, device=x.device)
    check(
        _lib.lib().chitu_hip_bf16_gemm_silu_add_norm(ptr(x), i64(x.stride(0)), ptr(add), i64(add.stride(0)), ptr(x_new), i64(K),
                                                     ptr(norm_weight), f32(eps), ptr(w13), ptr(out), i64(M), i64(inter), i64(K),
                                                     stream_ptr()),
        "bf16_linear_silu_add_norm",
    )
    return x_new, out


def silu_and_mul(x: torch.Tensor) -> torch.Tensor:
    require_cuda(x)
    assert x.dtype == torch.bfloat16 and x.is_contiguous() and x.shape[-1] % 16 == 0
    d = x.shape[-1] // 2
    out = torch.empty(*x.shape[:-1], d, dtype=torch.bfloat16, device=x.device)
    check(_lib.lib().chitu_hip_silu_and_mul(ptr(x), ptr(out), i64(x.numel() // (2 * d)), i64(d), stream_ptr()), "silu_and_mul")
    return out


_GATE_SPLITS = 16


_route_tickets = {}


def _route_ticket(device) -> torch.Tensor:
    key = (torch.device(device).index or 0, workspace._namespace)
    t = _route_tickets.get(key)
    if t is None:
        if torch.cuda.is_current_stream_capturing():
            raise RuntimeError("gate_deepseek_v3(align=...) must run once eagerly before graph capture")
        t = _route_tickets[key] = torch.zeros(1, dtype=torch.int32, device=device)
    return t


def gate_deepseek_v3(x, weight, bias, n_groups, topk_groups, topk, score_func, route_scale,
                     extra_expert_id: int = -1, extra_weight: float = 1.0, extra_count: int = 1, align=None,
                     logits_partials=None):
    require_cuda(weight)
    E = weight.shape[0]
    if logits_partials is not None:
        assert logits_partials.dtype == torch.float32 and logits_partials.dim() == 3 and logits_partials.is_contiguous()
        assert logits_partials.shape[2] == E
        M, dev = logits_partials.shape[1], logits_partials.device
    else:
        require_cuda(x)
        assert x.dtype == torch.bfloat16 and weight.dtype == torch.bfloat16 and x.is_contiguous() and weight.is_contiguous()
        M, K = x.shape
        dev = x.device
        if M < 256:
            splits = _GATE_SPLITS if K % (64 * _GATE_SPLITS) == 0 else 1
        else:
            tiles = ((M + 127) // 128) * ((E + 127) // 128)
            splits = 1
            while splits < 8 and tiles * splits < 256 and (K // 64) // (splits * 2) >= 4:
                splits *= 2
    cols = topk + (extra_count if extra_expert_id >= 0 else 0)
    w_out = torch.empty(M, cols, dtype=torch.bfloat16, device=dev)
    ids = torch.empty(M, cols, dtype=torch.int64, device=dev)
    lib = _lib.lib()
    if logits_partials is not None:
        logits, nparts = logits_partials, logits_partials.shape[0]
    elif splits > 1:
        part = torch.empty(splits, M, E, dtype=torch.float32, device=x.device)
        check(lib.chitu_hip_bf16_gemm(ptr(x), ptr(weight), ptr(None), i32(0), i64(M), i64(E), i64(K), i32(splits),
                                      ptr(part), stream_ptr()), "gate scores")
        logits, nparts = part, splits
    else:
        logits = bf16_linear(x, weight)
        nparts = 0
    sf = {"softmax": 0, "sigmoid": 1, "softmax_renorm": 2}[score_func]
    if align is None:
        check(
            lib.chitu_hip_gate_route(ptr(logits), i32(nparts), i64(M), i32(E), ptr(bias), i32(n_groups), i32(topk_groups),
                                     i32(topk), i32(sf), f32(route_scale), ptr(w_out), ptr(ids), i32(cols),
                                     i32(extra_expert_id), f32(extra_weight), i32(extra_count), stream_ptr()),
            "gate_route",
        )
        return w_out, ids
    a_experts, a_block, a_map = align
    cap = M * cols + a_experts * (a_block - 1)
    nblk = (cap + a_block - 1) // a_block
    sorted_ids = torch.empty(cap, dtype=torch.int32, device=dev)
    expert_ids = torch.empty(nblk, dtype=torch.int32, device=dev)
    npost = torch.empty(1, dtype=torch.int32, device=dev)
    cumsum = torch.empty(a_experts + 1, dtype=torch.int32, device=dev)
    if a_map is not None:
        assert a_map.dtype == torch.int32 and a_map.is_cuda and a_map.is_contiguous() and a_map.numel() >= a_experts
    check(
        lib.chitu_hip_gate_route_align(ptr(logits), i32(nparts), i64(M), i32(E), ptr(bias), i32(n_groups), i32(topk_groups),
                                       i32(topk), i32(sf), f32(route_scale), ptr(w_out), ptr(ids), i32(cols),
                                       i32(extra_expert_id), f32(extra_weight), i32(extra_count), i32(a_experts),
                                       i32(a_block), ptr(sorted_ids), i64(cap), ptr(expert_ids), i64(nblk), ptr(npost),
                                       ptr(cumsum), ptr(a_map), ptr(_route_ticket(dev)), stream_ptr()),
        "gate_route_align",
    )
    return w_out, ids, (sorted_ids, expert_ids, npost)


def mla_kv_prep(kv_in, q_pe, cos, sin, kv_norm_weight, eps, kv_cache, page_table, old_seq_lens):
    require_cuda(kv_in, q_pe, cos, sin, kv_norm_weight, kv_cache, page_table, old_seq_lens)
    assert kv_in.dtype == torch.bfloat16 and q_pe.dtype == torch.bfloat16 and kv_cache.dtype == torch.bfloat16
    assert kv_in.shape[-1] == 576 and kv_in.stride(-1) == 1 and q_pe.stride(-1) == 1 and q_pe.shape[-1] == 64
    assert kv_cache.is_contiguous() and kv_cache.shape[-1] == 576 and page_table.is_contiguous()
    assert cos.dtype == torch.float32 and cos.is_contiguous() and sin.is_contiguous()
    bs = kv_in.shape[0]
    check(
        _lib.lib().chitu_hip_mla_kv_prep(
            ptr(kv_in), i64(kv_in.stride(0)), ptr(q_pe), i64(q_pe.stride(0)), i64(q_pe.stride(1)), i32(q_pe.shape[1]),
            ptr(cos), ptr(sin), ptr(kv_norm_weight), f32(eps), ptr(kv_cache), i64(kv_cache.shape[0]),
            i32(kv_cache.shape[1]), ptr(page_table), i32(page_table.shape[1]), ptr(old_seq_lens), i32(bs), i32(512),
            i32(64), stream_ptr(),
        ),
        "mla_kv_prep",
    )


def mla_merge_absorb_uv_quant_fp8(partials, num_splits, batch, w, scale, scale_offset, scale_stride_h, scale_stride_k,
                                  tile_major: bool = False):
    require_cuda(partials, w, scale)
    assert w.element_size() == 1 and scale.dtype == torch.float32 and w.dim() == 3 and w.shape[1] == 128
    assert w.stride(2) == 1 and w.stride(1) == w.shape[2] and w.shape[2] == 512 and num_splits >= 2
    H = w.shape[0]
    assert partials.numel() * partials.element_size() >= batch * H * num_splits * (512 * 2 + 4)
    if tile_major:
        q, s = _tiled_buffers(batch, H * 128, w.device)
        fn = _lib.lib().chitu_hip_mla_merge_absorb_uv_quant_fp8_tm
    else:
        q = torch.empty(batch, H * 128, dtype=torch.float8_e4m3fn, device=w.device)
        s = torch.empty(batch, H, dtype=torch.float32, device=w.device)
        fn = _lib.lib().chitu_hip_mla_merge_absorb_uv_quant_fp8
    check(
        fn(ptr(partials), i32(num_splits), ptr(w), i64(w.stride(0)), ptr(scale), i64(scale_offset),
           i64(scale_stride_h), i64(scale_stride_k), ptr(q), ptr(s), i32(batch), i32(H), i32(512), stream_ptr()),
        "mla_merge_absorb_uv_quant_fp8",
    )
    return (TiledQuant(q, s, batch, H * 128), None) if tile_major else (q, s)


def embed_rope_gather(tokens, embed_weight, vocab_start, positions=None, cos_table=None, sin_table=None):
    require_cuda(tokens, embed_weight, positions, cos_table, sin_table)
    assert tokens.dtype == torch.int64 and tokens.dim() == 1 and tokens.is_contiguous()
    assert embed_weight.dtype == torch.bfloat16 and embed_weight.is_contiguous()
    bs, dim = tokens.shape[0], embed_weight.shape[1]
    h = torch.empty(bs, dim, dtype=torch.bfloat16, device=tokens.device)
    cos = sin = None
    half = rows = 0
    if positions is not None:
        assert positions.dtype == torch.int32 and positions.is_contiguous() and positions.numel() >= bs
        assert cos_table.dtype == torch.float32 and cos_table.is_contiguous() and sin_table.is_contiguous()
        rows, half = cos_table.shape
        cos = torch.empty(bs, half, dtype=torch.float32, device=tokens.device)
        sin = torch.empty(bs, half, dtype=torch.float32, device=tokens.device)
    check(
        _lib.lib().chitu_hip_embed_rope_gather(ptr(tokens), ptr(embed_weight), i64(vocab_start), i64(embed_weight.shape[0]),
                                               i32(dim), ptr(h), ptr(positions), ptr(cos_table), ptr(sin_table), i64(rows),
                                               i32(half), ptr(cos), ptr(sin), i32(bs), stream_ptr()),
        "embed_rope_gather",
    )
    return h, cos, sin


def mla_qkv_post(q_a_kv, q_lora_rank, q_norm_weight, q_eps, kv_norm_weight, kv_eps, cos, sin, kv_cache, page_table,
                 old_seq_lens):
    require_cuda(q_a_kv, q_norm_weight, kv_norm_weight, cos, sin, kv_cache, page_table, old_seq_lens)
    if q_a_kv.dtype == torch.float32:
        assert q_a_kv.dim() == 3 and q_a_kv.is_contiguous()
        nparts, bs, stride = q_a_kv.shape[0], q_a_kv.shape[1], q_a_kv.shape[2]
    else:
        assert q_a_kv.dtype == torch.bfloat16 and q_a_kv.dim() == 2 and q_a_kv.stride(1) == 1
        nparts, bs, stride = 0, q_a_kv.shape[0], q_a_kv.stride(0)
    assert q_a_kv.shape[-1] == q_lora_rank + 576 and kv_cache.dtype == torch.bfloat16 and kv_cache.shape[-1] == 576
    assert kv_cache.is_contiguous() and page_table.is_contiguous() and page_table.dtype == torch.int32
    assert cos.dtype == torch.float32 and cos.is_contiguous() and sin.is_contiguous() and old_seq_lens.dtype == torch.int32
    q = torch.empty(bs, q_lora_rank, dtype=torch.float8_e4m3fn, device=q_a_kv.device)
    s = torch.empty(bs, q_lora_rank // 128, dtype=torch.float32, device=q_a_kv.device)
    check(
        _lib.lib().chitu_hip_mla_qkv_post(
            ptr(q_a_kv), i32(nparts), i64(stride), i32(q_lora_rank), ptr(q_norm_weight), f32(q_eps), ptr(q), ptr(s),
            ptr(kv_norm_weight), f32(kv_eps), ptr(cos), ptr(sin), ptr(kv_cache), i64(kv_cache.shape[0]),
            i32(kv_cache.shape[1]), ptr(page_table), i32(page_table.shape[1]), ptr(old_seq_lens), i32(bs), i32(512),
            i32(64), stream_ptr(),
        ),
        "mla_qkv_post",
    )
    return q, s


def mla_q_proj_fits(bs: int, q_lora_rank: int) -> bool:
    return 0 < bs <= 32 and q_lora_rank % 128 == 0 and 128 <= q_lora_rank <= 2048


def mla_q_proj(q_a_kv, q_lora_rank, q_norm_weight, q_eps, wq_b, wq_b_scale, kv_norm_weight, kv_eps, cos, sin, kv_cache,
               page_table, old_seq_lens, out_dtype=None):
    require_cuda(q_a_kv, q_norm_weight, wq_b, wq_b_scale, kv_norm_weight, cos, sin, kv_cache, page_table, old_seq_lens)
    assert q_a_kv.dtype == torch.bfloat16 and q_a_kv.dim() == 2 and q_a_kv.stride(1) == 1
    bs = q_a_kv.shape[0]
    assert mla_q_proj_fits(bs, q_lora_rank), "use mla_qkv_post + fp8_gemm_deepseek_v3 for this shape"
    assert q_a_kv.shape[-1] == q_lora_rank + 576 and kv_cache.dtype == torch.bfloat16 and kv_cache.shape[-1] == 576
    assert kv_cache.is_contiguous() and page_table.is_contiguous() and page_table.dtype == torch.int32
    assert cos.dtype == torch.float32 and cos.is_contiguous() and sin.is_contiguous() and old_seq_lens.dtype == torch.int32
    assert wq_b.element_size() == 1 and wq_b.is_contiguous() and wq_b.shape[1] == q_lora_rank
    assert wq_b_scale.dtype == torch.float32 and wq_b_scale.is_contiguous()
    N = wq_b.shape[0]
    assert wq_b_scale.shape == ((N + 127) // 128, q_lora_rank // 128)
    out = torch.empty(bs, N, dtype=out_dtype or torch.get_default_dtype(), device=q_a_kv.device)
    check(
        _lib.lib().chitu_hip_mla_q_proj(
            ptr(q_a_kv), i64(q_a_kv.stride(0)), i32(q_lora_rank), ptr(q_norm_weight), f32(q_eps), ptr(wq_b), ptr(wq_b_scale),
            ptr(out), float_dtype_code(out.dtype), i64(N), ptr(kv_norm_weight), f32(kv_eps), ptr(cos), ptr(sin),
            ptr(kv_cache), i64(kv_cache.shape[0]), i32(kv_cache.shape[1]), ptr(page_table), i32(page_table.shape[1]),
            ptr(old_seq_lens), i32(bs), i32(512), i32(64), stream_ptr(),
        ),
        "mla_q_proj",
    )
    return out


def absorb_bmm_rope_fp8(x, w, scale, scale_offset, scale_stride_h, scale_stride_n, scale_stride_k, q_pe, cos, sin):
    require_cuda(x, w, scale, q_pe, cos, sin)
    assert x.dtype == torch.bfloat16 and w.element_size() == 1 and scale.dtype == torch.float32
    assert x.dim() == 3 and w.dim() == 3 and x.stride(-1) == 1 and w.stride(2) == 1 and w.stride(1) == w.shape[2]
    assert q_pe.dtype == torch.bfloat16 and q_pe.shape[-1] == 64 and q_pe.stride(-1) == 1
    assert cos.dtype == torch.float32 and cos.is_contiguous() and sin.is_contiguous()
# ... 140 lines not shown
```

Measured before the change: 205.5.

## Index MoE decode GEMMs by expert with per-expert slot tables built in gate

Adds a gate routing kernel that, for small batches (≤16 tokens), emits per-expert token counts and slot tables instead of the padded sorted-id alignment. New MoE gemm1 (with fused SiLU) and gemm2 (with fused quant) kernels launch one grid row per expert and read those tables directly. This replaces the block-size alignment and sort path and the padded M-blocks at decode. The new path only covers fp8 W8A8 without expert_map, and the grid is sized over all experts, so experts with no tokens still launch blocks that exit early.

```diff
diff --git a/chitu_amd/csrc/gate.hip b/chitu_amd/csrc/gate.hip
--- a/chitu_amd/csrc/gate.hip
+++ b/chitu_amd/csrc/gate.hip
@@ -1,5 +1,6 @@
 #include "common.h"
 #include "moe_align_device.h"
+#include "chitu_hip_ext7.h"
 
 namespace chitu {
 
@@ -445,6 +446,131 @@
     CHITU_PROBE_MARK(4);
 }
 
+template <int GS>
+__global__ __launch_bounds__(1024) void gate_route_expert_wg_kernel(
+    const void* __restrict__ logits, int S, int M, const bf16_t* __restrict__ bias, int n_groups, int topk_groups,
+    int topk, float route_scale, bf16_t* __restrict__ out_w, int64_t* __restrict__ out_ids, int out_stride,
+    int extra_id, float extra_w, int extra_n, int table_experts, MoeExpertTables tb) {
+    constexpr int E = 256;
+    extern __shared__ __attribute__((aligned(16))) int dyn_lds[];
+    const int nwaves = blockDim.x >> 6;
+    float* orig_lds = reinterpret_cast<float*>(dyn_lds);
+    int64_t* ids_lds = reinterpret_cast<int64_t*>(dyn_lds + nwaves * E);
+    int* align_lds = dyn_lds + nwaves * E + 2 * ((M * out_stride + 1) & ~1);
+    const int lane = threadIdx.x & 63, t = __builtin_amdgcn_readfirstlane(threadIdx.x >> 6);
+    CHITU_PROBE_MARK(0);
+    for (int i = (int)threadIdx.x; i < table_experts; i += (int)blockDim.x) align_lds[i] = 0;
+    __syncthreads();
+    if (t < M) {
+        float lg[4];
+        if (S == 0) {
+            const i32x2 raw = *reinterpret_cast<const i32x2*>((const bf16_t*)logits + (int64_t)t * E + lane * 4);
+            lg[0] = bf16_to_f32((bf16_t)((uint32_t)raw[0] & 0xffffu));
+            lg[1] = bf16_to_f32((bf16_t)((uint32_t)raw[0] >> 16));
+            lg[2] = bf16_to_f32((bf16_t)((uint32_t)raw[1] & 0xffffu));
+            lg[3] = bf16_to_f32((bf16_t)((uint32_t)raw[1] >> 16));
+        } else {
+            f32x4 v[16];
+#pragma unroll
+            for (int i = 0; i < 16; ++i)
+                v[i] = *reinterpret_cast<const f32x4*>((const float*)logits + ((int64_t)min(i, S - 1) * M + t) * E + lane * 4);
+            f32x4 a = f32x4{0.f, 0.f, 0.f, 0.f};
+#pragma unroll
+            for (int i = 0; i < 16; ++i)
+#pragma unroll
+                for (int c = 0; c < 4; ++c) a[c] += i < S ? v[i][c] : 0.f;
+#pragma unroll
+            for (int c = 0; c < 4; ++c) lg[c] = bf16r(a[c]);
+        }
+        float bv[4] = {0.f, 0.f, 0.f, 0.f};
+        if (bias) {
+            const i32x2 raw = *reinterpret_cast<const i32x2*>(bias + lane * 4);
+            bv[0] = bf16_to_f32((bf16_t)((uint32_t)raw[0] & 0xffffu));
+            bv[1] = bf16_to_f32((bf16_t)((uint32_t)raw[0] >> 16));
+            bv[2] = bf16_to_f32((bf16_t)((uint32_t)raw[1] & 0xffffu));
+            bv[3] = bf16_to_f32((bf16_t)((uint32_t)raw[1] >> 16));
+        }
+        float orig[4], sel[4];
+        uint32_t key[4];
+        if (lg[0] == 12345.678f) CHITU_PROBE_MARK(9);
+        CHITU_PROBE_MARK(1);
+#pragma unroll
+        for (int c = 0; c < 4; ++c) {
+            orig[c] = bf16r(1.0f / (1.0f + expf(-lg[c])));
+            sel[c] = bias ? bf16r(orig[c] + bv[c]) : orig[c];
+            key[c] = score_key(sel[c], lane * 4 + c);
+        }
+        *reinterpret_cast<f32x4*>(&orig_lds[t * E + lane * 4]) = f32x4{orig[0], orig[1], orig[2], orig[3]};
+        if (key[0] == 0xdeadbeefu) CHITU_PROBE_MARK(9);
+        CHITU_PROBE_MARK(5);
+        if (GS == 32) {
+            const uint32_t k1 = group8_max_u32(max(max(key[0], key[1]), max(key[2], key[3])));
+            uint32_t k2 = 0u;
+#pragma unroll
+            for (int c = 0; c < 4; ++c) k2 = max(k2, key[c] == k1 ? 0u : key[c]);
+            k2 = group8_max_u32(k2);
+            const float m1 = key_score(k1), m2 = key_score(k2);
+            const float mine = bias ? bf16r(m1 + m2) : m1;
+            const int grp = lane >> 3;
+            int rank = 0;
+#pragma unroll
+            for (int g2 = 0; g2 < 8; ++g2) {
+                const float o = __int_as_float(__builtin_amdgcn_readlane(__float_as_int(mine), g2 * 8));
+                rank += (g2 < n_groups) && ((o > mine) || (o == mine && g2 < grp));
+            }
+            if (rank >= topk_groups) {
+#pragma unroll
+                for (int c = 0; c < 4; ++c) key[c] = score_key(0.f, lane * 4 + c);
+            }
+        }
+        if (key[0] == 0xdeadbeefu) CHITU_PROBE_MARK(9);
+        CHITU_PROBE_MARK(6);
+        uint32_t mine_k = 0u;
+        for (int r = 0; r < topk; ++r) {
+            const uint32_t m = wave_max_u32_uniform(max(max(key[0], key[1]), max(key[2], key[3])));
+            if (lane == r) mine_k = m;
+#pragma unroll
+            for (int c = 0; c < 4; ++c)
+                if (key[c] == m) key[c] = 0u;
+        }
+        if (mine_k == 0xdeadbeefu) CHITU_PROBE_MARK(9);
+        CHITU_PROBE_MARK(7);
+        __builtin_amdgcn_fence(__ATOMIC_ACQ_REL, "wavefront");
+        __builtin_amdgcn_wave_barrier();
+        const int we = 0xffff - (int)(mine_k & 0xffffu);
+        const float ws = lane < topk ? orig_lds[t * E + (we & (E - 1))] : 0.f;
+        float sum = 0.f;
+        if (topk <= 16) {
+#pragma unroll
+            for (int i = 0; i < 16; ++i)
+                if (i < topk) sum += __int_as_float(__builtin_amdgcn_readlane(__float_as_int(ws), i));
+        } else {
+            for (int i = 0; i < topk; ++i) sum += __shfl(ws, i, 64);
+        }
+        if (lane < topk) {
+            float w = bf16r(ws / bf16r(sum));
+            w = bf16r(w * route_scale);
+            out_w[(int64_t)t * out_stride + lane] = f32_to_bf16(w);
+            out_ids[(int64_t)t * out_stride + lane] = we;
+            ids_lds[t * out_stride + lane] = we;
+            moe_align_small_mark(align_lds, we, t);
+        }
+        if (lane < extra_n && extra_id >= 0) {
+            out_ids[(int64_t)t * out_stride + topk + lane] = extra_id + lane;
+            out_w[(int64_t)t * out_stride + topk + lane] = f32_to_bf16(extra_w);
+            ids_lds[t * out_stride + topk + lane] = extra_id + lane;
+            moe_align_small_mark(align_lds, extra_id + lane, t);
+        }
+    }
+    CHITU_PROBE_MARK(2);
+    __syncthreads();
+    CHITU_PROBE_MARK(3);
+    const int tail_waves = min((int)(blockDim.x >> 6), max((table_experts + 63) >> 6, (M * out_stride + 63) >> 6));
+    if (t >= tail_waves) return;
+    moe_expert_tables_tail(ids_lds, M * out_stride, out_stride, table_experts, tb, align_lds);
+    CHITU_PROBE_MARK(4);
+}
+
 __device__ __forceinline__ uint32_t ordered_u32(float v) {
     const uint32_t b = __float_as_uint(v);
     return b ^ ((b & 0x80000000u) ? 0xffffffffu : 0x80000000u);
@@ -533,6 +659,80 @@
     moe_align_workgroup<int64_t>(ids_lds, (int64_t)M * out_stride, al.num_experts, al.block_size, al.sorted_ids,
                                  al.sorted_cap, al.expert_ids, al.expert_cap, al.num_post_pad, al.cumsum, 1,
                                  al.expert_map, align_lds, sort_waves * 64);
+}
+
+__global__ __launch_bounds__(1024) void gate_route_expert_wg_softmax_kernel(
+    const void* __restrict__ logits, int S, int M, int E, const bf16_t* __restrict__ bias, int topk, float route_scale,
+    bf16_t* __restrict__ out_w, int64_t* __restrict__ out_ids, int out_stride, int extra_id, float extra_w, int extra_n,
+    int renorm, int table_experts, MoeExpertTables tb) {
+    extern __shared__ __attribute__((aligned(16))) int dyn_lds[];
+    int64_t* ids_lds = reinterpret_cast<int64_t*>(dyn_lds);
+    int* align_lds = dyn_lds + 2 * ((M * out_stride + 1) & ~1);
+    const int lane = threadIdx.x & 63, t = __builtin_amdgcn_readfirstlane(threadIdx.x >> 6);
+    for (int i = (int)threadIdx.x; i < table_experts; i += (int)blockDim.x) align_lds[i] = 0;
+    __syncthreads();
+    if (t < M) {
+        const bool act = lane < E;
+        const int ec = act ? lane : E - 1;
+        float logit;
+        if (S == 0) {
+            logit = bf16_to_f32(((const bf16_t*)logits)[(int64_t)t * E + ec]);
+        } else {
+            float v[16];
+#pragma unroll
+            for (int i = 0; i < 16; ++i) v[i] = ((const float*)logits)[((int64_t)min(i, S - 1) * M + t) * E + ec];
+            float a = 0.f;
+#pragma unroll
+            for (int i = 0; i < 16; ++i) a += i < S ? v[i] : 0.f;
+            logit = bf16r(a);
+        }
+        const float bv = bias ? bf16_to_f32(bias[ec]) : 0.f;
+        if (!act) logit = -INFINITY;
+        const float m = wave_reduce_max(logit);
+        const float ex = act ? expf(logit - m) : 0.f;
+        const float sum = wave_reduce_sum(ex);
+        const float orig = ex / sum;
+        const float sel = bias ? orig + bv : orig;
+        uint32_t key = act ? ordered_u32(sel) : 0u;
+        int my_e = 0;
+        float my_w = 0.f;
+        for (int r = 0; r < topk; ++r) {
+            const uint32_t mk = wave_max_u32_uniform(key);
+            const unsigned long long hit = __ballot(act && key == mk);
+            const int win = __builtin_amdgcn_readfirstlane(__ffsll((long long)hit) - 1);
+            const float w = __int_as_float(__builtin_amdgcn_readlane(__float_as_int(orig), win));
+            if (lane == r) {
+                my_e = win;
+                my_w = w;
+            }
+            if (lane == win) key = 0u;
+        }
+        float w = my_w;
+        if (renorm) {
+            float s2 = 0.f;
+#pragma unroll
+            for (int i = 0; i < 16; ++i)
+                if (i < topk) s2 += __int_as_float(__builtin_amdgcn_readlane(__float_as_int(my_w), i));
+            w = w / s2;
+        }
+        w = w * route_scale;
+        if (lane < topk) {
+            out_w[(int64_t)t * out_stride + lane] = f32_to_bf16(w);
+            out_ids[(int64_t)t * out_stride + lane] = my_e;
+            ids_lds[t * out_stride + lane] = my_e;
+            moe_align_small_mark(align_lds, my_e, t);
+        }
+        if (lane < extra_n && extra_id >= 0) {
+            out_ids[(int64_t)t * out_stride + topk + lane] = extra_id + lane;
+            out_w[(int64_t)t * out_stride + topk + lane] = f32_to_bf16(extra_w);
+            ids_lds[t * out_stride + topk + lane] = extra_id + lane;
+            moe_align_small_mark(align_lds, extra_id + lane, t);
+        }
+    }
+    __syncthreads();
+    const int tail_waves = min((int)(blockDim.x >> 6), max((table_experts + 63) >> 6, (M * out_stride + 63) >> 6));
+    if (t >= tail_waves) return;
+    moe_expert_tables_tail(ids_lds, M * out_stride, out_stride, table_experts, tb, align_lds);
 }
 
 }
@@ -660,4 +860,55 @@
                              extra_weight, extra_count, al, stream);
 }
 
+extern "C" int chitu_ext7_gate_route_experts(const void* logits, int32_t num_partials, int64_t tokens, int32_t num_experts,
+                                             const void* bias_bf16, int32_t n_groups, int32_t topk_groups, int32_t topk,
+                                             int32_t score_func, float route_scale, void* out_weights_bf16, int64_t* out_ids,
+                                             int32_t out_stride, int32_t extra_expert_id, float extra_weight,
+                                             int32_t extra_count, int32_t table_experts, int32_t* count, int32_t* slot_of,
+                                             void* stream) {
+    using namespace chitu;
+    CHITU_REQUIRE(logits && out_weights_bf16 && out_ids && count && slot_of && tokens >= 0);
+    CHITU_REQUIRE(num_experts >= 1 && num_experts <= 1024 && topk >= 1 && topk <= num_experts && topk <= 64);
+    CHITU_REQUIRE(n_groups >= 1 && n_groups <= 64 && num_experts % n_groups == 0);
+    CHITU_REQUIRE(topk_groups >= 1 && topk_groups <= n_groups && num_partials >= 0);
+    CHITU_REQUIRE(extra_count >= 0 && extra_count <= 32 && table_experts >= 1 && table_experts <= 1024);
+    CHITU_REQUIRE(score_func >= 0 && score_func <= 2);
+    CHITU_REQUIRE(out_stride == topk + (extra_expert_id >= 0 ? extra_count : 0));
+    CHITU_REQUIRE(num_experts <= table_experts &&
+                  (extra_expert_id < 0 || (extra_expert_id >= num_experts && extra_expert_id + extra_count <= table_experts)));
+    if (tokens > 16 || num_partials > 16) return CHITU_ERR_UNSUPPORTED;
+    if (tokens == 0) return CHITU_OK;
+    const int wg_threads = 64 * max((int)tokens, (table_experts + 63) / 64);
+    if (wg_threads > 1024 || tokens * out_stride > wg_threads) return CHITU_ERR_UNSUPPORTED;
+    const size_t ids_ints = 2 * (((size_t)tokens * out_stride + 1) & ~(size_t)1);
+    hipStream_t st = (hipStream_t)stream;
+    const MoeExpertTables tb{count, slot_of};
+    const int gs = n_groups > 1 ? num_experts / n_groups : 0;
+    const int threads = ((table_experts + 63) / 64) * 64;
+    if (score_func == 1 && num_experts == 256 && (gs == 0 || gs == 32) && (threads / 64) * topk <= 64 &&
+        ((threads / 64) * topk) % 4 == 0 && n_groups <= 32) {
+        const size_t wg_lds = sizeof(int) * ((size_t)(wg_threads / 64) * 256 + ids_ints + (size_t)table_experts);
+        CHITU_REQUIRE(wg_lds <= 64 * 1024);
+#define LAUNCHX(GSV)                                                                                          \
+    hipLaunchKernelGGL(gate_route_expert_wg_kernel<GSV>, dim3(1), dim3(wg_threads), wg_lds, st, logits,        \
+                       (int)num_partials, (int)tokens, (const bf16_t*)bias_bf16, (int)n_groups, (int)topk_groups, \
+                       (int)topk, route_scale, (bf16_t*)out_weights_bf16, out_ids, (int)out_stride,           \
+                       (int)extra_expert_id, extra_weight, (int)extra_count, (int)table_experts, tb)
+        if (gs == 32) LAUNCHX(32);
+        else LAUNCHX(0);
+#undef LAUNCHX
+        CHITU_RETURN_LAUNCH_STATUS();
+    }
+    if (num_experts <= 64 && (score_func == 0 || score_func == 2) && n_groups <= 1 && topk <= 16) {
+        const size_t wg_lds = sizeof(int) * (ids_ints + (size_t)table_experts);
+        CHITU_REQUIRE(wg_lds <= 64 * 1024);
+        hipLaunchKernelGGL(gate_route_expert_wg_softmax_kernel, dim3(1), dim3(wg_threads), wg_lds, st, logits, (int)num_partials,
+                           (int)tokens, (int)num_experts, (const bf16_t*)bias_bf16, (int)topk, route_scale,
+                           (bf16_t*)out_weights_bf16, out_ids, (int)out_stride, (int)extra_expert_id, extra_weight,
+                           (int)extra_count, score_func == 2 ? 1 : 0, (int)table_experts, tb);
+        CHITU_RETURN_LAUNCH_STATUS();
+    }
+    return CHITU_ERR_UNSUPPORTED;
+}
+
 CHITU_PROBE_READER(gate)
diff --git a/chitu_amd/csrc/moe.hip b/chitu_amd/csrc/moe.hip
--- a/chitu_amd/csrc/moe.hip
+++ b/chitu_amd/csrc/moe.hip
@@ -1,5 +1,6 @@
 #include "common.h"
 #include "gemm_common.h"
+#include "chitu_hip_ext7.h"
 #ifndef CHITU_MOE_PROBE_MASK
 #define CHITU_MOE_PROBE_MASK 0
 #endif
@@ -222,6 +223,102 @@
     if (wave_id == 0 && g == 0) hs[(size_t)slot * (I >> 7) + blockIdx.x] = sc;
 }
 
+template <int WK, int D>
+__global__ __launch_bounds__(64 * WK) void moe_gemm1_silu_expert_kernel(
+    const fp8_t* __restrict__ Xq, const float* __restrict__ Xs, const fp8_t* __restrict__ W,
+    const float* __restrict__ Ws, const int32_t* __restrict__ count, const int32_t* __restrict__ slot_of,
+    bf16_t* __restrict__ out, int numel, int topk, int I, int K) {
+    __shared__ float red[WK > 1 ? WK * 512 : 1];
+    const int e = blockIdx.y;
+    const int cnt = count[e];
+    int slot = slot_of[e * 16 + (threadIdx.x & 15)];
+    asm volatile("" : "+v"(slot));
+    if (cnt <= 0) return;
+    const int lane = threadIdx.x & 63;
+    const int wave = __builtin_amdgcn_readfirstlane(threadIdx.x >> 6);
+    const int j = lane & 15, g = lane >> 4;
+    const int n0 = blockIdx.x * 16;
+    const int N = 2 * I;
+    const int KB = K >> 7;
+    const bool valid = j < cnt && (unsigned)slot < (unsigned)numel;
+    f32x4 ag = f32x4{0.f, 0.f, 0.f, 0.f}, au = f32x4{0.f, 0.f, 0.f, 0.f};
+    {
+        const int kb0 = KB * wave / WK, kb1 = KB * (wave + 1) / WK;
+        const int slot0 = __builtin_amdgcn_readfirstlane(slot);
+        const int token = (valid ? slot : (int)min((unsigned)slot0, (unsigned)(numel - 1))) / topk;
+        const fp8_t* xp = Xq + (size_t)token * K + g * 16;
+        const float* xsp = Xs + (size_t)token * KB;
+        const fp8_t* Wb = W + (size_t)e * N * K;
+        const fp8_t *gp0, *gp1, *up0, *up1;
+        w8_lane_ptrs(Wb, n0, N, K, j, g, gp0, gp1);
+        w8_lane_ptrs(Wb, I + n0, N, K, j, g, up0, up1);
+        const float* wsb = Ws + (size_t)e * ((N + 127) >> 7) * KB;
+        const float* wsgp = wsb + (size_t)(n0 >> 7) * KB;
+        const float* wsup = wsb + (size_t)((I + n0) >> 7) * KB;
+        auto load = [&](MoeStage2& st, int kb) {
+            const int off = kb << 7;
+            st.wg.w[0] = __builtin_nontemporal_load(reinterpret_cast<const i32x4*>(gp0 + off));
+            st.wg.w[1] = __builtin_nontemporal_load(reinterpret_cast<const i32x4*>(gp1 + off));
+            st.wu.w[0] = __builtin_nontemporal_load(reinterpret_cast<const i32x4*>(up0 + off));
+            st.wu.w[1] = __builtin_nontemporal_load(reinterpret_cast<const i32x4*>(up1 + off));
+            st.x[0] = *reinterpret_cast<const i32x4*>(xp + off);
+            st.x[1] = *reinterpret_cast<const i32x4*>(xp + off + 64);
+            st.xs = xsp[kb];
+            st.wsg = wsgp[kb];
+            st.wsu = wsup[kb];
+        };
+        auto compute = [&](const MoeStage2& st) {
+            const f32x4 bg = w8a8_block_dot(st.wg, st.x[0], st.x[1]);
+            const f32x4 bu = w8a8_block_dot(st.wu, st.x[0], st.x[1]);
+#pragma unroll
+            for (int r = 0; r < 4; ++r) {
+                ag[r] += (bg[r] * st.xs) * st.wsg;
+                au[r] += (bu[r] * st.xs) * st.wsu;
+            }
+        };
+        MoeStage2 ring[D];
+#pragma unroll
+        for (int d = 0; d < D; ++d)
+            if (kb0 + d < kb1) load(ring[d], kb0 + d);
+        for (int kb = kb0; kb < kb1; kb += D) {
+#pragma unroll
+            for (int d = 0; d < D; ++d) {
+                if (kb + d < kb1) {
+                    compute(ring[d]);
+                    if (kb + d + D < kb1) load(ring[d], kb + d + D);
+                }
+            }
+        }
+    }
+    if (WK > 1) {
+        *reinterpret_cast<f32x4*>(&red[(wave * 128 + lane) * 4]) = ag;
+        *reinterpret_cast<f32x4*>(&red[(wave * 128 + 64 + lane) * 4]) = au;
+        __syncthreads();
+        if (wave != 0) return;
+        ag = f32x4{0.f, 0.f, 0.f, 0.f};
+        au = f32x4{0.f, 0.f, 0.f, 0.f};
+#pragma unroll
+        for (int w = 0; w < WK; ++w) {
+            const f32x4 vg = *reinterpret_cast<const f32x4*>(&red[(w * 128 + lane) * 4]);
+            const f32x4 vu = *reinterpret_cast<const f32x4*>(&red[(w * 128 + 64 + lane) * 4]);
+#pragma unroll
+            for (int r = 0; r < 4; ++r) {
+                ag[r] += vg[r];
+                au[r] += vu[r];
+            }
+        }
+    }
+    if (!valid) return;
+    f32x4 h;
+#pragma unroll
+    for (int r = 0; r < 4; ++r) {
+        const float gv = round_bf16(ag[r]), uv = round_bf16(au[r]);
+        const float sl = round_bf16(gv / (1.0f + expf(-gv)));
+        h[r] = round_bf16(sl * uv);
+    }
+    moe_store_tile(out + (size_t)slot * I, n0, g, I, h, 1.0f);
+}
+
 __global__ __launch_bounds__(256) void moe_silu_quant_kernel(const bf16_t* __restrict__ c1,
                                                              fp8_t* __restrict__ q,
                                                              float* __restrict__ s, int64_t rows,
@@ -354,6 +451,112 @@
             }
         return;
     }
+    const int row = valid ? slot : 0;
+    const bf16_t* hrow = Hb + (size_t)row * I;
+    i32x4 hraw[HPW][2];
+#pragma unroll
+    for (int q = 0; q < HPW; ++q) {
+        const int hb = min(wave + 4 * q, 2 * KB - 1);
+        hraw[q][0] = *reinterpret_cast<const i32x4*>(hrow + hb * 64 + g * 16);
+        hraw[q][1] = *reinterpret_cast<const i32x4*>(hrow + hb * 64 + g * 16 + 8);
+    }
+    const int last_tile = (N - 1) >> 4;
+    const fp8_t* We = W + (size_t)e * N * I;
+    W8Frag wf[ROUNDS > 1 ? 2 : 1][NT][KB];
+    auto load_round = [&](W8Frag (&dst)[NT][KB], int r) {
+#pragma unroll
+        for (int t = 0; t < NT; ++t) {
+            const int n0 = min(tile_of(r) + t, last_tile) * 16;
+            const fp8_t *wp0, *wp1;
+            w8_lane_ptrs(We, n0, N, I, j, g, wp0, wp1);
+#pragma unroll
+            for (int kb = 0; kb < KB; ++kb) {
+                dst[t][kb].w[0] = __builtin_nontemporal_load(reinterpret_cast<const i32x4*>(wp0 + (kb << 7)));
+                dst[t][kb].w[1] = __builtin_nontemporal_load(reinterpret_cast<const i32x4*>(wp1 + (kb << 7)));
+            }
+        }
+    };
+    load_round(wf[0], 0);
+    const float rw = (mul_weight && valid) ? moe_routed_weight(topk_w, w_dt, slot) : 1.0f;
+    float h[HPW][16];
+#pragma unroll
+    for (int q = 0; q < HPW; ++q) {
+        const int hb = wave + 4 * q;
+        float amax = 0.f;
+#pragma unroll
+        for (int i = 0; i < 16; ++i) {
+            const uint32_t u = (uint32_t)hraw[q][i >> 3][(i >> 1) & 3];
+            h[q][i] = (i & 1) ? __uint_as_float(u & 0xffff0000u) : __uint_as_float(u << 16);
+            amax = __builtin_fmaxf(amax, __builtin_fabsf(h[q][i]));
+        }
+        amax = __builtin_fmaxf(amax, __shfl_xor(amax, 16, 64));
+        amax = __builtin_fmaxf(amax, __shfl_xor(amax, 32, 64));
+        if (g == 0 && hb < 2 * KB) amax_lds[hb][j] = amax;
+    }
+    __syncthreads();
+#pragma unroll
+    for (int q = 0; q < HPW; ++q) {
+        const int hb = wave + 4 * q;
+        if (hb < 2 * KB) {
+            const float sc = __builtin_fmaxf(__builtin_fmaxf(amax_lds[hb & ~1][j], amax_lds[hb | 1][j]), eps) / 448.0f;
+            float lo[8], hi[8];
+#pragma unroll
+            for (int i = 0; i < 8; ++i) {
+                lo[i] = h[q][i];
+                hi[i] = h[q][8 + i];
+            }
+            const i32x2 a = quant8_fp8<true>(lo, sc), b = quant8_fp8<true>(hi, sc);
+            xq_lds[hb][lane] = i32x4{a[0], a[1], b[0], b[1]};
+        }
+    }
+    __syncthreads();
+    i32x4 x[KB][2];
+    float xs[KB];
+#pragma unroll
+    for (int kb = 0; kb < KB; ++kb) {
+        x[kb][0] = xq_lds[2 * kb][lane];
+        x[kb][1] = xq_lds[2 * kb + 1][lane];
+        xs[kb] = __builtin_fmaxf(__builtin_fmaxf(amax_lds[2 * kb][j], amax_lds[2 * kb + 1][j]), eps) / 448.0f;
+    }
+    const float* wse = Ws + (size_t)e * ((N + 127) >> 7) * KB;
+#pragma unroll
+    for (int r = 0; r < ROUNDS; ++r) {
+        if (r + 1 < ROUNDS) load_round(wf[(r + 1) & 1], r + 1);
+#pragma unroll
+        for (int t = 0; t < NT; ++t) {
+            const int n0 = (tile_of(r) + t) * 16;
+            f32x4 acc = f32x4{0.f, 0.f, 0.f, 0.f};
+            const float* wsp = wse + (size_t)(min(n0, N - 1) >> 7) * KB;
+#pragma unroll
+            for (int kb = 0; kb < KB; ++kb) {
+                const f32x4 blk = w8a8_block_dot(wf[r & 1][t][kb], x[kb][0], x[kb][1]);
+                const float ws = wsp[kb];
+#pragma unroll
+                for (int rr = 0; rr < 4; ++rr) acc[rr] += (blk[rr] * xs[kb]) * ws;
+            }
+            if (valid && n0 < N) moe_store_tile(out + (size_t)slot * N, n0, g, N, acc, rw);
+        }
+    }
+}
+
+template <int KB, int NT, int ROUNDS>
+__global__ __launch_bounds__(256) void moe_gemm2_q_expert_kernel(
+    const bf16_t* __restrict__ Hb, const fp8_t* __restrict__ W, const float* __restrict__ Ws,
+    const int32_t* __restrict__ count, const int32_t* __restrict__ slot_of, const void* __restrict__ topk_w, int w_dt,
+    bf16_t* __restrict__ out, int numel, int N, int mul_weight, float eps) {
+    constexpr int I = KB * 128;
+    constexpr int HPW = (2 * KB + 3) / 4;
+    __shared__ float amax_lds[2 * KB][16];
+    __shared__ i32x4 xq_lds[2 * KB][64];
+    const int e = blockIdx.y;
+    const int cnt = count[e];
+    int slot = slot_of[e * 16 + (threadIdx.x & 15)];
+    asm volatile("" : "+v"(slot));
+    if (cnt <= 0) return;
+    const int lane = threadIdx.x & 63, wave = __builtin_amdgcn_readfirstlane(threadIdx.x >> 6);
+    const int j = lane & 15, g = lane >> 4;
+    const bool valid = j < cnt && (unsigned)slot < (unsigned)numel;
+    auto tile_of = [&](int r) { return ((blockIdx.x * ROUNDS + r) * 4 + wave) * NT; };
     const int row = valid ? slot : 0;
     const bf16_t* hrow = Hb + (size_t)row * I;
     i32x4 hraw[HPW][2];
@@ -717,6 +920,73 @@
     CHITU_RETURN_LAUNCH_STATUS();
 }
 
+extern "C" int chitu_ext7_moe_gemm1_silu_fp8_experts(const void* a_fp8, const float* a_scale, const void* w1_fp8,
+                                                     const float* w1_scale, const int32_t* count, const int32_t* slot_of,
+                                                     void* h_bf16, int64_t numel, int32_t topk, int64_t inter_size,
+                                                     int64_t K, int64_t num_experts, int64_t max_mblocks, void* stream) {
+    using namespace chitu;
+    CHITU_REQUIRE(a_fp8 && a_scale && w1_fp8 && w1_scale && count && slot_of && h_bf16);
+    CHITU_REQUIRE(numel >= 0 && topk >= 1 && inter_size >= 16 && K >= 128 && max_mblocks >= 0);
+    CHITU_REQUIRE(num_experts >= 1 && num_experts <= 65535);
+    if (K % 128 != 0 || inter_size % 16 != 0) return CHITU_ERR_UNSUPPORTED;
+    if (numel > 16 * (int64_t)topk) return CHITU_ERR_UNSUPPORTED;
+    if (numel == 0 || max_mblocks == 0) return CHITU_OK;
+    const int n_tiles = (int)(inter_size / 16);
+    const int64_t wgs = 2 * (int64_t)n_tiles * (numel < max_mblocks ? numel : max_mblocks);
+    const int KB = (int)(K / 128);
+    int WK = wgs <= 640 ? 8 : wgs <= 1536 ? 4 : wgs <= 3200 ? 2 : 1;
+    debug_override(kOptMoeGemm1WK, WK);
+    while (WK > 1 && WK > KB) WK >>= 1;
+    hipStream_t st = (hipStream_t)stream;
+    const dim3 grid((unsigned)n_tiles, (unsigned)num_experts);
+#define LAUNCH1X(WKV, DV)                                                                                            \
+    hipLaunchKernelGGL((moe_gemm1_silu_expert_kernel<WKV, DV>), grid, dim3(64 * WKV), 0, st, (const fp8_t*)a_fp8, a_scale, \
+                       (const fp8_t*)w1_fp8, w1_scale, count, slot_of, (bf16_t*)h_bf16, (int)numel, (int)topk,       \
+                       (int)inter_size, (int)K)
+    if (WK == 8) LAUNCH1X(8, 2);
+    else if (WK == 4) LAUNCH1X(4, 2);
+    else if (WK == 2) LAUNCH1X(2, 3);
+    else if (WK == 1) LAUNCH1X(1, 3);
+    else return CHITU_ERR_BAD_ARG;
+#undef LAUNCH1X
+    CHITU_RETURN_LAUNCH_STATUS();
+}
+
+extern "C" int chitu_ext7_moe_gemm2_quant_fp8_experts(const void* h_bf16, const void* w2_fp8, const float* w2_scale,
+                                                      const int32_t* count, const int32_t* slot_of,
+                                                      const void* topk_weights, int weights_dtype,
+                                                      int32_t mul_routed_weight, void* out_bf16, int64_t numel, int64_t N,
+                                                      int64_t inter_size, int64_t num_experts, int64_t max_mblocks,
+                                                      float eps, void* stream) {
+    using namespace chitu;
+    CHITU_REQUIRE(h_bf16 && w2_fp8 && w2_scale && count && slot_of && out_bf16 && (topk_weights || !mul_routed_weight));
+    CHITU_REQUIRE(numel >= 0 && N >= 1 && inter_size >= 128 && max_mblocks >= 0);
+    CHITU_REQUIRE(weights_dtype >= 0 && weights_dtype <= 2 && num_experts >= 1 && num_experts <= 65535);
+    if (inter_size % 128 != 0 || inter_size > 512) return CHITU_ERR_UNSUPPORTED;
+    if (numel == 0 || max_mblocks == 0) return CHITU_OK;
+    hipStream_t st = (hipStream_t)stream;
+    const int n_tiles = (int)((N + 15) / 16);
+    const int KB = (int)(inter_size / 128);
+    const int64_t mbs = numel < max_mblocks ? numel : max_mblocks;
+#define LAUNCH2X(KBV, NTV, RV)                                                                          \
+    hipLaunchKernelGGL((moe_gemm2_q_expert_kernel<KBV, NTV, RV>),                                       \
+                       dim3((unsigned)((n_tiles + 4 * NTV * RV - 1) / (4 * NTV * RV)), (unsigned)num_experts), \
+                       dim3(256), 0, st, (const bf16_t*)h_bf16, (const fp8_t*)w2_fp8, w2_scale, count, slot_of, \
+                       topk_weights, weights_dtype, (bf16_t*)out_bf16, (int)numel, (int)N, (int)mul_routed_weight, eps)
+    const bool many = (int64_t)n_tiles * mbs > 50000;
+    switch (KB) {
+        case 1: LAUNCH2X(1, 2, 1); break;
+        case 2:
+            if (many) LAUNCH2X(2, 2, 4);
+            else LAUNCH2X(2, 2, 1);
+            break;
+        case 3: LAUNCH2X(3, 2, 1); break;
+        default: LAUNCH2X(4, 2, 1); break;
+    }
+#undef LAUNCH2X
+    CHITU_RETURN_LAUNCH_STATUS();
+}
+
 extern "C" int chitu_hip_moe_sum(const void* c3_bf16, void* out_bf16, int64_t tokens, int32_t topk,
                                  int64_t N, void* stream) {
     using namespace chitu;
diff --git a/chitu_amd/csrc/moe_align_device.h b/chitu_amd/csrc/moe_align_device.h
--- a/chitu_amd/csrc/moe_align_device.h
+++ b/chitu_amd/csrc/moe_align_device.h
@@ -193,4 +193,23 @@
     }
 }
 
-}
+struct MoeExpertTables {
+    int32_t* count;
+    int32_t* slot_of;
+};
+
+__device__ __forceinline__ void moe_expert_tables_tail(const int64_t* __restrict__ ids_lds, int numel, int stride, int E,
+                                                       const MoeExpertTables& tb, const int* tmask) {
+    const int tid = threadIdx.x;
+    if (tid < E) tb.count[tid] = __popc((unsigned)tmask[tid] & 0xffffu);
+    if (tid < numel) {
+        const int e = (int)ids_lds[tid];
+        const int t = tid / stride;
+        if (e >= 0 && e < E && t < 16) {
+            const int r = __popc((unsigned)tmask[e] & ((1u << t) - 1u));
+            tb.slot_of[e * 16 + r] = (int32_t)tid;
+        }
+    }
+}
+
+}
diff --git a/chitu_amd/deepseek_v3.py b/chitu_amd/deepseek_v3.py
--- a/chitu_amd/deepseek_v3.py
+++ b/chitu_amd/deepseek_v3.py
@@ -363,6 +363,10 @@
     return tokens <= _ROUTE_ALIGN_MAX_TOKENS and os.environ.get("CHITU_ROUTE_ALIGN", "1") != "0"
 
 
+def _moe_by_expert_enabled() -> bool:
+    return os.environ.get("CHITU_MOE_BY_EXPERT", "0") == "1"
+
+
 class GateDeepSeekV3(torch.nn.Module):
 
     def __init__(self, args, device=None):
@@ -373,10 +377,15 @@
         self.bias = (torch.nn.Parameter(torch.empty(args.n_routed_experts, dtype=torch.bfloat16, device=device), requires_grad=False)
                      if args.has_gate_bias() else None)
 
-    def forward(self, x, extra_expert_id: int = -1, extra_count: int = 1, align=None, logits_partials=None):
+    def forward(self, x, extra_expert_id: int = -1, extra_count: int = 1, align=None, logits_partials=None, by_expert=None):
+        extra = {} if by_expert is None else {"by_expert": by_expert}
         return ops.gate_deepseek_v3(x, self.weight, self.bias, self.n_groups, self.topk_groups, self.topk,
                                     self.score_func, self.route_scale, extra_expert_id=extra_expert_id,
-                                    extra_count=extra_count, align=align, logits_partials=logits_partials)
+                                    extra_count=extra_count, align=align, logits_partials=logits_partials, **extra)
+
+    def by_expert_supported(self, tokens: int, table_experts: int, cols: int, num_partials: int = 0) -> bool:
+        return ops.route_by_expert_supported(tokens, self.weight.shape[0], self.n_groups, self.topk, self.score_func,
+                                             table_experts, cols, num_partials)
 
 
 class MoEDeepSeekV3(torch.nn.Module):
@@ -423,9 +432,16 @@
         nr, ns = self.n_routed, self.n_shared
         if self.moe_world_size > 1:
             return self.forward_expert_parallel(x, x_quant)
-        align = (nr + ns, fused_moe._MOE_BLOCK_M, None) if _route_align_enabled(x.shape[0]) else None
-        routed = (self.gate(x, extra_expert_id=nr, extra_count=ns, align=align, logits_partials=logits_partials) if ns >= 1
-                  else self.gate(x, align=align, logits_partials=logits_partials))
+        bs = x.shape[0]
+        by_expert = (not self.mxfp4 and _moe_by_expert_enabled() and _route_align_enabled(bs)
+                     and fused_moe.by_expert_eligible(bs, self.inter)
+                     and self.gate.by_expert_supported(bs, nr + ns, self.gate.topk + ns,
+                                                       0 if logits_partials is None else logits_partials.shape[0]))
+        align = (nr + ns, fused_moe._MOE_BLOCK_M, None) if _route_align_enabled(bs) and not by_expert else None
+        kw = dict(align=align, logits_partials=logits_partials)
+        if by_expert:
+            kw["by_expert"] = nr + ns
+        routed = self.gate(x, extra_expert_id=nr, extra_count=ns, **kw) if ns >= 1 else self.gate(x, **kw)
         weights, indices = routed[0], routed[1]
         aligned = routed[2] if len(routed) > 2 else None
         return fused_moe.fused_experts(
diff --git a/chitu_amd/fused_moe.py b/chitu_amd/fused_moe.py
--- a/chitu_amd/fused_moe.py
+++ b/chitu_amd/fused_moe.py
@@ -1,6 +1,6 @@
 
 import os
-from typing import List, Optional, Tuple
+from typing import List, NamedTuple, Optional, Tuple
 
 import torch
 
@@ -124,6 +124,19 @@
 _MOE_MXFP4_TILED_MIN_TOKENS = int(os.environ.get("CHITU_MOE_MXFP4_TILED_MIN_TOKENS", "512"))
 _MOE_BF16_TILED_MIN_TOKENS = int(os.environ.get("CHITU_MOE_BF16_TILED_MIN_TOKENS", "0"))
 
+
+
+_MOE_BY_EXPERT_MAX_TOKENS = 16
+
+
+class ExpertTables(NamedTuple):
+    count: torch.Tensor
+    slot_of: torch.Tensor
+
+
+def by_expert_eligible(num_tokens, I, expert_map=None) -> bool:
+    return (1 <= num_tokens <= _MOE_BY_EXPERT_MAX_TOKENS and I % 128 == 0 and I <= 512 and expert_map is None
+            and os.environ.get("CHITU_MOE_FUSE_SILU", "1") != "0")
 
 
 def _takes_tiled(num_tokens, numel, global_num_experts, I, Nout, aligned, min_tokens=None):
@@ -203,6 +216,11 @@
     bf16_tiled_min_tokens: Optional[int] = None,
     use_mxfp4_w4a8: bool = False,
 ):
+    expert_tables = aligned if isinstance(aligned, ExpertTables) else None
+    if expert_tables is not None:
+        if use_mxfp4_w4a8 or use_int8_w8a8 or not use_fp8_w8a8 or soft_fp8:
+            raise ValueError("ExpertTables: only the fp8 W8A8 experts have the launches indexed by expert")
+        aligned = None
     if use_mxfp4_w4a8:
         if activation != "silu":
             raise ValueError(f"Unsupported FusedMoe activation: {activation}")
@@ -259,7 +277,11 @@
     def rnd(n):
         return (n + 255) // 256 * 256
 
+    if expert_tables is not None and not by_expert_eligible(num_tokens, I, expert_map):
+        raise ValueError("ExpertTables: needs at most 16 tokens, an expert width of 128 .. 512 in whole 128-blocks and no expert_map")
     tiled = _takes_tiled(num_tokens, numel, global_num_experts, I, Nout, aligned)
+    if expert_tables is not None:
+        tiled = False
     block_m = _MOE_TILED_BLOCK_M if tiled else _MOE_BLOCK_M
     cap = numel + global_num_experts * (block_m - 1)
     nblk = ceil_div(cap, block_m)
@@ -284,7 +306,12 @@
     st = stream_ptr()
     max_mblocks = min(nblk, numel)
 
-    if aligned is None:
+    if expert_tables is not None:
+        t_count, t_slots = expert_tables
+        require_cuda(t_count, t_slots)
+        assert t_count.dtype == torch.int32 and t_slots.dtype == torch.int32 and t_count.is_contiguous() and t_slots.is_contiguous()
+        assert t_count.numel() == global_num_experts == E and t_slots.numel() == 16 * E, "tables must range over the stacked experts"
+    elif aligned is None:
         emap = _expert_map_i32(expert_map, global_num_experts, dev)
         check(
             lib.chitu_hip_moe_align_block_size_mapped(
@@ -315,7 +342,23 @@
         assert aq.is_contiguous() and as_.is_contiguous() and aq.numel() == num_tokens * K
         assert as_.dtype == torch.float32 and as_.numel() == num_tokens * KB
         a1q_p, a1s_p = ptr(aq), ptr(as_)
-    if tiled:
+    if expert_tables is not None:
+        check(
+            lib.chitu_ext7_moe_gemm1_silu_fp8_experts(
+                a1q_p, a1s_p, ptr(w1), ptr(w1_scale), ptr(t_count), ptr(t_slots), P("c1"),
+                i64(numel), i32(topk), i64(I), i64(K), i64(E), i64(max_mblocks), st,
+            ),
+            "moe gemm1 (by expert, silu fused)",
+        )
+        check(
+            lib.chitu_ext7_moe_gemm2_quant_fp8_experts(
+                P("c1"), ptr(w2), ptr(w2_scale), ptr(t_count), ptr(t_slots), ptr(topk_weights),
+                float_dtype_code(topk_weights.dtype), i32(1), P("c3"), i64(numel), i64(Nout), i64(I), i64(E),
+                i64(max_mblocks), f32(1e-10), st,
+            ),
+            "moe gemm2 (by expert, quant fused)",
+        )
+    elif tiled:
         assert nblk <= 65535
         check(
             lib.chitu_hip_moe_gemm1_silu_fp8_tiled(
diff --git a/chitu_amd/ops.py b/chitu_amd/ops.py
--- a/chitu_amd/ops.py
+++ b/chitu_amd/ops.py
@@ -778,9 +778,25 @@
     return t
 
 
+_ROUTE_BY_EXPERT_MAX_TOKENS = 16
+
+
+def route_by_expert_supported(tokens, num_experts, n_groups, topk, score_func, table_experts, cols, num_partials=0) -> bool:
+    if not (1 <= tokens <= _ROUTE_BY_EXPERT_MAX_TOKENS and num_partials <= 16 and num_experts <= table_experts <= 1024):
+        return False
+    threads = 64 * max(tokens, (table_experts + 63) // 64)
+    if threads > 1024 or tokens * cols > threads:
+        return False
+    waves = (table_experts + 63) // 64
+    gs = num_experts // n_groups if n_groups > 1 else 0
+    if score_func == "sigmoid":
+        return num_experts == 256 and gs in (0, 32) and waves * topk <= 64 and (waves * topk) % 4 == 0 and n_groups <= 32 and topk <= 64
+    return score_func in ("softmax", "softmax_renorm") and num_experts <= 64 and n_groups <= 1 and topk <= 16
+
+
 def gate_deepseek_v3(x, weight, bias, n_groups, topk_groups, topk, score_func, route_scale,
                      extra_expert_id: int = -1, extra_weight: float = 1.0, extra_count: int = 1, align=None,
-                     logits_partials=None):
+                     logits_partials=None, by_expert=None):
     require_cuda(weight)
     E = weight.shape[0]
     if logits_partials is not None:
@@ -814,6 +830,21 @@
         logits = bf16_linear(x, weight)
         nparts = 0
     sf = {"softmax": 0, "sigmoid": 1, "softmax_renorm": 2}[score_func]
+    if by_expert is not None:
+        assert align is None, "by_expert replaces align"
+        t_experts = int(by_expert)
+        count = torch.empty(t_experts, dtype=torch.int32, device=dev)
+        slot_of = torch.empty(t_experts, 16, dtype=torch.int32, device=dev)
+        check(
+            lib.chitu_ext7_gate_route_experts(ptr(logits), i32(nparts), i64(M), i32(E), ptr(bias), i32(n_groups), i32(topk_groups),
+                                              i32(topk), i32(sf), f32(route_scale), ptr(w_out), ptr(ids), i32(cols),
+                                              i32(extra_expert_id), f32(extra_weight), i32(extra_count), i32(t_experts),
+                                              ptr(count), ptr(slot_of), stream_ptr()),
+            "gate_route_experts",
+        )
+        from .fused_moe import ExpertTables
+
+        return w_out, ids, ExpertTables(count, slot_of)
     if align is None:
         check(
             lib.chitu_hip_gate_route(ptr(logits), i32(nparts), i64(M), i32(E), ptr(bias), i32(n_groups), i32(topk_groups),
diff --git a/include/chitu_hip_ext7.h b/include/chitu_hip_ext7.h
--- /dev/null
+++ b/include/chitu_hip_ext7.h
@@ -0,0 +1,30 @@
+#ifndef CHITU_HIP_EXT7_H
+#define CHITU_HIP_EXT7_H
+
+#include "chitu_hip.h"
+
+#ifdef __cplusplus
+extern "C" {
+#endif
+
+#define CHITU_HIP_EXT7_VERSION 1
+
+int chitu_ext7_gate_route_experts(const void* logits, int32_t num_partials, int64_t tokens, int32_t num_experts,
+                                  const void* bias_bf16, int32_t n_groups, int32_t topk_groups, int32_t topk,
+                                  int32_t score_func, float route_scale, void* out_weights_bf16, int64_t* out_ids,
+                                  int32_t out_stride, int32_t extra_expert_id, float extra_weight, int32_t extra_count,
+                                  int32_t table_experts, int32_t* count, int32_t* slot_of, void* stream);
+int chitu_ext7_moe_gemm1_silu_fp8_experts(const void* a_fp8, const float* a_scale, const void* w1_fp8, const float* w1_scale,
+                                          const int32_t* count, const int32_t* slot_of, void* h_bf16, int64_t numel,
+                                          int32_t topk, int64_t inter_size, int64_t K, int64_t num_experts,
+                                          int64_t max_mblocks, void* stream);
+int chitu_ext7_moe_gemm2_quant_fp8_experts(const void* h_bf16, const void* w2_fp8, const float* w2_scale, const int32_t* count,
+                                           const int32_t* slot_of, const void* topk_weights, int weights_dtype,
+                                           int32_t mul_routed_weight, void* out_bf16, int64_t numel, int64_t N,
+                                           int64_t inter_size, int64_t num_experts, int64_t max_mblocks, float eps,
+                                           void* stream);
+
+#ifdef __cplusplus
+}
+#endif
+#endif
```

New measurement: 205.5, median of 2. No clear change (+0.0%).
